# aarchiiive/diff-unet-amos

Measured on NVIDIA B200. Metric: 96^3 patches/s (DDIM-10), higher is better.
Workload: dtype fp16 (fp32 accumulate; encoder in split-bf16)

## Files before the change

### diff-unet-amos_b200/csrc/conv3d_ref.cuh

```cuda
#pragma once
#include <cuda_bf16.h>
#include <cuda_runtime.h>

#include "elementwise.cuh"

namespace dunet {

template <bool HF>
__global__ void __launch_bounds__(128) conv3d_ref_kernel(const __nv_bfloat16* __restrict__ src0, int c0, int chunks0,
                                                         const __nv_bfloat16* __restrict__ src1, int c1, int chunks1,
                                                         const float* __restrict__ w ,
                                                         __nv_bfloat16* __restrict__ out, int cout, int out_chunks,
                                                         int D, int H, int W, int batch, int rot) {
  const long long vox = (long long)D * H * W;
  const int och = (cout + 7) / 8;
  const int cin = c0 + c1;
  const long long total = (long long)batch * och * vox;
  for (long long i = blockIdx.x * (long long)blockDim.x + threadIdx.x; i < total;
       i += (long long)gridDim.x * blockDim.x) {
    const long long v = i % vox;
    const int oc = (int)((i / vox) % och);
    const int n = (int)(i / (vox * och));
    const int x = (int)(v % W), y = (int)((v / W) % H), z = (int)(v / ((long long)W * H));
    float acc[8];
#pragma unroll
    for (int j = 0; j < 8; ++j) acc[j] = 0.f;
    for (int tz = 0; tz < 3; ++tz) {
      const int zz = z + tz - 1;
      if (zz < 0 || zz >= D) continue;
      for (int ty = 0; ty < 3; ++ty) {
        const int yy = y + ty - 1;
        if (yy < 0 || yy >= H) continue;
        for (int tx = 0; tx < 3; ++tx) {
          const int xx = x + tx - 1;
          if (xx < 0 || xx >= W) continue;
          const int tap = (tz * 3 + ty) * 3 + tx;
          const long long sv = ((long long)zz * H + yy) * W + xx;
          for (int ci = 0; ci < cin; ci += 8) {
            const bool second = ci >= c0;
            const BF8* sp = second ? reinterpret_cast<const BF8*>(src1) + ((long long)n * chunks1 + (ci - c0) / 8) * vox
                                   : reinterpret_cast<const BF8*>(src0) + ((long long)n * chunks0 + ci / 8) * vox;
            float xi[8];
            bf8_to_float<HF>(sp[sv], xi);
#pragma unroll
            for (int k = 0; k < 8; ++k) {
              if (ci + k < cin) {
#pragma unroll
                for (int j = 0; j < 8; ++j) {
                  if (oc * 8 + j >= cout) continue;
                  const float wv =
                      round_16<HF>(w[((long long)(oc * 8 + j) * cin + (rot ? (ci + k + 1) % c0 : ci + k)) * 27 + tap]);
                  acc[j] = fmaf(xi[k], wv, acc[j]);
                }
              }
            }
          }
        }
      }
    }
    reinterpret_cast<BF8*>(out)[((long long)n * out_chunks + oc) * vox + v] = float_to_bf8<HF>(acc);
  }
}

}
```

### diff-unet-amos_b200/csrc/conv3d_tc64.cuh

```cuda
#pragma once
#include <cuda.h>
#include <cuda_bf16.h>
#include <cuda_runtime.h>

#include <type_traits>

#include "conv3d_tc.cuh"

namespace dunet {

template <int CB_CH, int ZT>
struct ConvTc64 {
  static constexpr int HX = CONV_TX + 2, HY = CONV_TY + 2;
  static constexpr int KCH = CB_CH / 8;
  static constexpr int KC = CB_CH / 16;
  static constexpr int PLANE_BYTES = KCH * HY * HX * 16;
  static constexpr int A_LBO = HY * HX * 16, A_SBO = HX * 16;
  static constexpr int NROWS = 192;
  static constexpr int W_UNIT_BYTES = KCH * NROWS * 16;
  static constexpr int B_LBO = NROWS * 16, B_SBO = 128;
  static constexpr int PLANES = ZT + 2;
  static constexpr int A_SLOTS = CB_CH == 32 ? 2 * PLANES + 1 : PLANES + 1;
  static constexpr int W_SLOTS = CB_CH == 32 ? 4 : 2;
  static constexpr int ACC_COLS = ZT * 64;
  static constexpr int TMEM_COLS = 512;
  static constexpr int RED_BYTES = 4 * 128 * 4;
  static constexpr int SMEM_BYTES = A_SLOTS * PLANE_BYTES + W_SLOTS * W_UNIT_BYTES + RED_BYTES + 1024 + 512;
  static constexpr int XFORM_WARPS = 8;
  static constexpr int THREADS_FUSED = CONV_THREADS + XFORM_WARPS * 32;
  static_assert(2 * ACC_COLS <= 512, "double-buffered accumulators exceed TMEM");
  static_assert(SMEM_BYTES <= 232448, "shared memory budget");
};

struct ConvTc64Args {
  const __nv_bfloat16* w;
  __nv_bfloat16* out;
  __nv_bfloat16* out_lo;
  float* stats;
  ConvSegs segs;
  int D, H, W;
  int tiles_x, tiles_y, tiles_z, batch;
  const float* in_affine;
  const float* in_bias;
  int in_bias_n_stride;
  float slope;
};

template <class F>
__device__ __forceinline__ void for_each_tile(int tiles_per_n, int batch, F&& f) {
  const int G = gridDim.x, shift = tiles_per_n % G;
  for (int n = 0; n < batch; ++n) {
    const int r = (int)((blockIdx.x + (long long)G * batch - (long long)n * shift) % G);
    for (int lin = r; lin < tiles_per_n; lin += G) f(n, lin);
  }
}

template <int CB_CH, int ZT, bool FUSE, bool H>
__global__ void __launch_bounds__(FUSE ? ConvTc64<CB_CH, ZT>::THREADS_FUSED : CONV_THREADS, 1)
conv3d_tc64_kernel(const __grid_constant__ CUtensorMap tmap0, const __grid_constant__ CUtensorMap tmap1,
                   const __grid_constant__ CUtensorMap tmap2, const __grid_constant__ CUtensorMap tmap3, ConvTc64Args a) {
  using Cfg = ConvTc64<CB_CH, ZT>;
  extern __shared__ uint8_t smem_raw[];
  const uint32_t smem_base = (smem_u32(smem_raw) + 1023u) & ~1023u;
  const uint32_t a_smem = smem_base;
  const uint32_t w_smem = a_smem + Cfg::A_SLOTS * Cfg::PLANE_BYTES;
  const uint32_t red_smem = w_smem + Cfg::W_SLOTS * Cfg::W_UNIT_BYTES;
  const uint32_t bars = red_smem + Cfg::RED_BYTES;
  const uint32_t a_full = bars, a_empty = bars + 8 * Cfg::A_SLOTS;
  const uint32_t w_full = bars + 16 * Cfg::A_SLOTS, w_empty = w_full + 8 * Cfg::W_SLOTS;
  const uint32_t acc_full = w_empty + 8 * Cfg::W_SLOTS;
  const uint32_t acc_empty = acc_full + 16;
  const uint32_t tmem_slot = acc_empty + 16;
  const uint32_t a_ready = tmem_slot + 8;
  static_assert(16 * Cfg::A_SLOTS + 16 * Cfg::W_SLOTS + 32 + 8 + 8 * Cfg::A_SLOTS <= 512, "barrier block");
  float* red = reinterpret_cast<float*>(smem_raw + (red_smem - smem_u32(smem_raw)));

  const int warp = threadIdx.x >> 5, lane = threadIdx.x & 31;
  const int ncb = a.segs.ncb;
  const int tiles_per_n = a.tiles_x * a.tiles_y * a.tiles_z;

  if (threadIdx.x == 0) {
    for (int i = 0; i < Cfg::A_SLOTS; ++i) { mbar_init(a_full + 8 * i, 1); mbar_init(a_empty + 8 * i, 1); mbar_init(a_ready + 8 * i, Cfg::XFORM_WARPS); }
    for (int i = 0; i < Cfg::W_SLOTS; ++i) { mbar_init(w_full + 8 * i, 1); mbar_init(w_empty + 8 * i, 1); }
    for (int i = 0; i < 2; ++i) { mbar_init(acc_full + 8 * i, 1); mbar_init(acc_empty + 8 * i, 4); }
    fence_mbar_init();
  }
  if (warp == 2) {
    tmem_alloc(tmem_slot, Cfg::TMEM_COLS);
    tmem_relinquish();
  }
  if (warp == 0 && lane == 0) {
    tma_prefetch_desc(&tmap0);
    if (a.segs.n > 1) tma_prefetch_desc(&tmap1);
    if (a.segs.n > 2) { tma_prefetch_desc(&tmap2); tma_prefetch_desc(&tmap3); }
  }
  tc_fence_before();
  __syncthreads();
  tc_fence_after();
  pdl_wait();
  uint32_t tmem_base;
  asm volatile("ld.shared.u32 %0, [%1];" : "=r"(tmem_base) : "r"(tmem_slot));

  if (warp == 0) {
    if (elect_one_sync()) {
      const CUtensorMap* const tms[4] = {&tmap0, &tmap1, &tmap2, &tmap3};
      int u = 0;
      for_each_tile(tiles_per_n, a.batch, [&](int n, int lin) {
        int t = lin;
        const int tix = t % a.tiles_x; t /= a.tiles_x;
        const int tiy = t % a.tiles_y; t /= a.tiles_y;
        const int tiz = t;
        const int x0 = tix * CONV_TX, y0 = tiy * CONV_TY, z0 = tiz * ZT;
        for (int cb = 0; cb < ncb; ++cb) {
          int ti, chunk0, chunks;
          conv_seg_lookup(a.segs, cb, Cfg::KCH, ti, chunk0, chunks);
          const CUtensorMap* tm = tms[ti];
          const int c3 = n * chunks + chunk0;
          for (int p = 0; p < Cfg::PLANES; ++p, ++u) {
            const int slot = u % Cfg::A_SLOTS, it = u / Cfg::A_SLOTS;
            if (it > 0) mbar_wait(a_empty + 8 * slot, (it - 1) & 1);
            mbar_arrive_expect_tx(a_full + 8 * slot, Cfg::PLANE_BYTES);
            tma_load_4d(a_smem + slot * Cfg::PLANE_BYTES, tm, a_full + 8 * slot, (x0 - 1) * 8, y0 - 1, z0 + p - 1, c3);
          }
        }
      });
    }
  } else if (warp == 1) {
    if (elect_one_sync()) {
      int w = 0;
      for_each_tile(tiles_per_n, a.batch, [&](int, int) {
        for (int i = 0; i < ncb * 9; ++i, ++w) {
          const int slot = w % Cfg::W_SLOTS, it = w / Cfg::W_SLOTS;
          if (it > 0) mbar_wait(w_empty + 8 * slot, (it - 1) & 1);
          mbar_arrive_expect_tx(w_full + 8 * slot, Cfg::W_UNIT_BYTES);
          bulk_load_1d(w_smem + slot * Cfg::W_UNIT_BYTES,
                       reinterpret_cast<const uint8_t*>(a.w) + (size_t)i * Cfg::W_UNIT_BYTES, Cfg::W_UNIT_BYTES,
                       w_full + 8 * slot);
        }
      });
    }
  } else if (warp == 2) {
    if (elect_one_sync()) {
      const uint64_t a_desc0 = make_smem_desc(a_smem, Cfg::A_LBO, Cfg::A_SBO);
      const uint64_t b_desc0 = make_smem_desc(w_smem, Cfg::B_LBO, Cfg::B_SBO);
      const uint32_t a_lo0 = (uint32_t)a_desc0, a_hi = (uint32_t)(a_desc0 >> 32);
      const uint32_t b_lo0 = (uint32_t)b_desc0, b_hi = (uint32_t)(b_desc0 >> 32);
      static_assert((Cfg::W_SLOTS & (Cfg::W_SLOTS - 1)) == 0, "W_SLOTS must be a power of two");
      int u0 = 0, w = 0, li = 0;
      for_each_tile(tiles_per_n, a.batch, [&](int, int) {
        const int buf = li & 1, use = li >> 1;
        if (use > 0) { mbar_wait(acc_empty + 8 * buf, (use - 1) & 1); tc_fence_after(); }
        const uint32_t acc = tmem_base + buf * Cfg::ACC_COLS;
        for (int cb = 0; cb < ncb; ++cb, u0 += Cfg::PLANES) {
          uint32_t pl_lo[Cfg::PLANES], pl_bar[Cfg::PLANES];
          uint32_t par[Cfg::PLANES];
#pragma unroll
          for (int p = 0; p < Cfg::PLANES; ++p) {
            const int u = u0 + p, slot = u % Cfg::A_SLOTS;
            pl_lo[p] = a_lo0 + slot * (Cfg::PLANE_BYTES >> 4);
            pl_bar[p] = 8 * slot;
            par[p] = (u / Cfg::A_SLOTS) & 1;
          }
          auto tap = [&](auto kind, int tyx, bool first_cb) {
            constexpr int KIND = decltype(kind)::value;
            const int ws = w & (Cfg::W_SLOTS - 1);
            mbar_wait(w_full + 8 * ws, (w / Cfg::W_SLOTS) & 1);
            tc_fence_after();
            const uint32_t tap16 = (tyx / 3) * Cfg::HX + (tyx % 3);
            const uint32_t bl_u = b_lo0 + ws * (Cfg::W_UNIT_BYTES >> 4);
#pragma unroll
            for (int p = 0; p < Cfg::PLANES; ++p) {
              if constexpr (KIND == 0) {
                mbar_wait((FUSE ? a_ready : a_full) + pl_bar[p], par[p]);
                tc_fence_after();
              }
              constexpr int dummy = 0; (void)dummy;
              const int slab_lo = p >= 2 ? p - 2 : 0, slab_hi = p < ZT ? p : ZT - 1;
              const int nblk = slab_hi - slab_lo + 1;
              const int row0 = (2 - (p - slab_lo)) * 64;
              const uint32_t al_p = pl_lo[p] + tap16, bl_p = bl_u + row0;
#pragma unroll
              for (int k = 0; k < Cfg::KC; ++k) {
                const uint32_t al = al_p + k * 2 * (Cfg::A_LBO >> 4), bl = bl_p + k * 2 * (Cfg::B_LBO >> 4);
                if (KIND == 0 && k == 0 && first_cb) {
#pragma unroll
                  for (int i = 0; i < nblk; ++i) {
                    const int sl = slab_lo + i, tz = p - sl;
                    umma_bf16_lh(acc + sl * 64, al, a_hi, bl + i * 64, b_hi, make_idesc_16(128, 64, H), tz != 0 ? 1u : 0u);
                  }
                } else {
                  umma_bf16_lh(acc + slab_lo * 64, al, a_hi, bl, b_hi, make_idesc_16(128, 64 * nblk, H), 1u);
                }
              }
              if constexpr (KIND == 2) umma_commit(a_empty + pl_bar[p]);
            }
            umma_commit(w_empty + 8 * ws);
            ++w;
          };
          tap(std::integral_constant<int, 0>{}, 0, cb == 0);
#pragma unroll 1
          for (int tyx = 1; tyx < 8; ++tyx) tap(std::integral_constant<int, 1>{}, tyx, false);
          tap(std::integral_constant<int, 2>{}, 8, false);
        }
        umma_commit(acc_full + 8 * buf);
        ++li;
      });
    }
    __syncwarp();
    pdl_trigger();
  } else if (FUSE && warp >= 7) {
    constexpr int LPC = Cfg::XFORM_WARPS * 32 / Cfg::KCH;
    constexpr int NPOS = Cfg::HY * Cfg::HX;
    constexpr int NV = (NPOS + LPC - 1) / LPC;
    const int tt = threadIdx.x - 7 * 32, chunk = tt / LPC, l0 = tt % LPC;
    uint8_t* const a_gen = smem_raw + (a_smem - smem_u32(smem_raw)) + chunk * (NPOS * 16) + l0 * 16;
    int pos_y[NV], pos_x[NV];
#pragma unroll
    for (int j = 0; j < NV; ++j) {
      const int i = l0 + j * LPC;
      pos_y[j] = i < NPOS ? i / Cfg::HX : 1 << 20;
      pos_x[j] = i % Cfg::HX;
    }
    float sc[8], sh[8], bi[8];
    int u = 0;
    for_each_tile(tiles_per_n, a.batch, [&](int n, int lin) {
      int t = lin;
      const int tix = t % a.tiles_x; t /= a.tiles_x;
      const int tiy = t % a.tiles_y; t /= a.tiles_y;
      const int tiz = t;
      const int x0 = tix * CONV_TX - 1, y0 = tiy * CONV_TY - 1, z0 = tiz * ZT - 1;
      uint32_t mask = 0;
#pragma unroll
      for (int j = 0; j < NV; ++j) {
        const int gy = y0 + pos_y[j], gx = x0 + pos_x[j];
        if (gy >= 0 && gy < a.H && gx >= 0 && gx < a.W) mask |= 1u << j;
      }
      for (int cb = 0; cb < ncb; ++cb) {
        {
          const int gch = cb * Cfg::KCH + chunk;
          const float4* src = reinterpret_cast<const float4*>(a.in_affine + ((long long)n * (ncb * Cfg::KCH) + gch) * 16);
#ifdef DUNET_AFFINE_LDG
          const float4 s0 = __ldg(src), s1 = __ldg(src + 1), h0 = __ldg(src + 2), h1 = __ldg(src + 3);
#else
          const float4 s0 = __ldcg(src), s1 = __ldcg(src + 1), h0 = __ldcg(src + 2), h1 = __ldcg(src + 3);
#endif
          sc[0] = s0.x; sc[1] = s0.y; sc[2] = s0.z; sc[3] = s0.w; sc[4] = s1.x; sc[5] = s1.y; sc[6] = s1.z; sc[7] = s1.w;
          sh[0] = h0.x; sh[1] = h0.y; sh[2] = h0.z; sh[3] = h0.w; sh[4] = h1.x; sh[5] = h1.y; sh[6] = h1.z; sh[7] = h1.w;
#pragma unroll
          for (int j = 0; j < 8; ++j) bi[j] = a.in_bias ? __ldg(a.in_bias + (long long)n * a.in_bias_n_stride + gch * 8 + j) : 0.f;
        }
        for (int p = 0; p < Cfg::PLANES; ++p, ++u) {
          const int slot = u % Cfg::A_SLOTS;
          mbar_wait(a_full + 8 * slot, (u / Cfg::A_SLOTS) & 1);
          const int gz = z0 + p;
          if (gz >= 0 && gz < a.D) {
            uint8_t* const pl = a_gen + slot * Cfg::PLANE_BYTES;
            constexpr int G = 6;
#pragma unroll
            for (int j0 = 0; j0 < NV; j0 += G) {
              BF8 v[G];
#pragma unroll
              for (int j = 0; j < G; ++j)
                if (j0 + j < NV && (mask >> (j0 + j) & 1u)) v[j] = *reinterpret_cast<const BF8*>(pl + (j0 + j) * (LPC * 16));
#pragma unroll
              for (int j = 0; j < G; ++j)
                if (j0 + j < NV && (mask >> (j0 + j) & 1u)) {
                  float f[8];
                  bf8_to_float<H>(v[j], f);
                  norm_apply(f, sc, sh, bi, a.slope);
                  *reinterpret_cast<BF8*>(pl + (j0 + j) * (LPC * 16)) = float_to_bf8<H>(f);
                }
            }
          }
          fence_proxy_async_smem();
          __syncwarp();
          if (lane == 0) mbar_arrive(a_ready + 8 * slot);
        }
      }
    });
  } else {
    const int q = warp & 3;
    const int r = q * 32 + lane;
    const long long vox = (long long)a.D * a.H * a.W;
    float run[4] = {0.f, 0.f, 0.f, 0.f};
    int cur_n = 0;
// ... 76 lines not shown
```

### diff-unet-amos_b200/csrc/dunet.cu

```cuda
#include <algorithm>
#include <atomic>
#include <cmath>
#include <cstdarg>
#include <cstdio>
#include <cstdlib>
#include <cstring>
#include <mutex>
#include <set>
#include <string>
#include <unordered_map>
#include <vector>

#include <cuda.h>
#include <cuda_bf16.h>
#include <cuda_runtime.h>

#include "../../include/dunet.h"
#include "conv3d_ref.cuh"
#include "conv3d_tc.cuh"
#include "conv3d_tc64.cuh"
#include "conv3d_flat.cuh"
#include "deconv2_tc.cuh"
#include "elementwise.cuh"
#include "surface.cuh"
// ... 58 lines not shown
}
static int prof_end_(Prof* pr, cudaStream_t st) {
  if (!pr || !pr->on) return 0;
  CUDA_TRY(cudaEventRecord(pr->recs[pr->used].b, st));
  ++pr->used;
  return 0;
}
#define prof_begin(tag, st) prof_begin_(prof_of(p), tag, st)
#define prof_end(st) prof_end_(prof_of(p), st)
#define PROF_ON (prof_of(p)->on)

template <typename... KArgs, typename... Args>
static void launch_k(void (*kern)(KArgs...), dim3 grid, dim3 block, size_t smem, cudaStream_t st, Args&&... args) {
  cudaLaunchConfig_t cfg;
  memset(&cfg, 0, sizeof cfg);
  cfg.gridDim = grid; cfg.blockDim = block; cfg.dynamicSmemBytes = smem; cfg.stream = st;
  cudaLaunchAttribute at[1];
  at[0].id = cudaLaunchAttributeProgrammaticStreamSerialization;
  at[0].val.programmaticStreamSerializationAllowed = 1;
  cfg.attrs = at; cfg.numAttrs = 1;
  (void)cudaLaunchKernelEx(&cfg, kern, std::forward<Args>(args)...);
}

static inline int pad_to(int v, int m) { return (v + m - 1) / m * m; }
static inline int grid_for(long long total, int threads, int cap = 148 * 16) {
  long long b = (total + threads - 1) / threads;
  if (b > cap) b = cap;
  if (b < 1) b = 1;
  return (int)b;
}
static bool aligned16(const void* p) { return (reinterpret_cast<uintptr_t>(p) & 15u) == 0; }

typedef CUresult (*EncodeTiledFn)(CUtensorMap*, CUtensorMapDataType, cuuint32_t, void*, const cuuint64_t*,
                                  const cuuint64_t*, const cuuint32_t*, const cuuint32_t*, CUtensorMapInterleave,
                                  CUtensorMapSwizzle, CUtensorMapL2promotion, CUtensorMapFloatOOBfill);
static EncodeTiledFn g_encode = nullptr;

static int load_driver_entry() {
  if (g_encode) return 0;
  void* fn = nullptr;
  cudaDriverEntryPointQueryResult q;
  CUDA_TRY(cudaGetDriverEntryPoint("cuTensorMapEncodeTiled", &fn, cudaEnableDefault, &q));
  if (!fn || q != cudaDriverEntryPointSuccess) return fail(DUNET_E_CUDA, "cuTensorMapEncodeTiled not available");
  g_encode = reinterpret_cast<EncodeTiledFn>(fn);
  return 0;
}

static int make_act_tmap(CUtensorMap* m, const bf16* base, int planes, int D, int H, int W, int kch, int halo) {
  TRY(load_driver_entry());
  cuuint64_t dims[4] = {(cuuint64_t)W * 8, (cuuint64_t)H, (cuuint64_t)D, (cuuint64_t)planes};
  cuuint64_t strides[3] = {(cuuint64_t)W * 16, (cuuint64_t)H * W * 16, (cuuint64_t)D * H * W * 16};
  cuuint32_t box[4] = {(cuuint32_t)(CONV_TX + 2 * halo) * 8, (cuuint32_t)(CONV_TY + 2 * halo), 1, (cuuint32_t)kch};
  cuuint32_t estr[4] = {1, 1, 1, 1};
  CUresult r = g_encode(m, CU_TENSOR_MAP_DATA_TYPE_BFLOAT16, 4, const_cast<bf16*>(base), dims, strides, box, estr,
                        CU_TENSOR_MAP_INTERLEAVE_NONE, CU_TENSOR_MAP_SWIZZLE_NONE, CU_TENSOR_MAP_L2_PROMOTION_L2_256B,
                        CU_TENSOR_MAP_FLOAT_OOB_FILL_NONE);
  if (r != CUDA_SUCCESS) return fail(DUNET_E_CUDA, "cuTensorMapEncodeTiled failed with CUresult %d (W=%d H=%d D=%d planes=%d)",
                                     (int)r, W, H, D, planes);
  return 0;
}

static int make_flat_tmap(CUtensorMap* m, const bf16* base, int planes, int D, int H, int W, int hx, int ty, int halo = 1) {
  TRY(load_driver_entry());
  cuuint64_t dims[4] = {(cuuint64_t)W * 8, (cuuint64_t)H, (cuuint64_t)D, (cuuint64_t)planes};
  cuuint64_t strides[3] = {(cuuint64_t)W * 16, (cuuint64_t)H * W * 16, (cuuint64_t)D * H * W * 16};
  cuuint32_t box[4] = {(cuuint32_t)hx * 8, (cuuint32_t)(ty + 2 * halo), 1, 8};
  cuuint32_t estr[4] = {1, 1, 1, 1};
  CUresult r = g_encode(m, CU_TENSOR_MAP_DATA_TYPE_BFLOAT16, 4, const_cast<bf16*>(base), dims, strides, box, estr,
                        CU_TENSOR_MAP_INTERLEAVE_NONE, CU_TENSOR_MAP_SWIZZLE_NONE, CU_TENSOR_MAP_L2_PROMOTION_L2_256B,
                        CU_TENSOR_MAP_FLOAT_OOB_FILL_NONE);
  if (r != CUDA_SUCCESS) return fail(DUNET_E_CUDA, "cuTensorMapEncodeTiled (flat) failed with CUresult %d (W=%d H=%d D=%d planes=%d hx=%d ty=%d)",
                                     (int)r, W, H, D, planes, hx, ty);
  return 0;
}

__device__ __forceinline__ bf16 weight_part(float v, int part, int fp16) {
  if (fp16) {
    const __half h = __float2half_rn(v);
    return *reinterpret_cast<const bf16*>(&h);
  }
  const bf16 hi = __float2bfloat16_rn(v);
  return part < 2 ? hi : __float2bfloat16_rn(v - __bfloat162float(hi));
}
__global__ void pack_conv_w_kernel(const float* __restrict__ w, bf16* __restrict__ out, int coutr, int cinr, int c0r,
                                   int c0p, int c1r, int cb_ch, int n_tile, int ncb, int n_tiles, int rot, int parts, int fp16, int triple) {
  const int kch = cb_ch / 8;
  const int ncb1 = ncb / parts;
  const long long total = (long long)n_tiles * ncb * 27 * kch * n_tile * 8;
  for (long long i = blockIdx.x * (long long)blockDim.x + threadIdx.x; i < total;
       i += (long long)gridDim.x * blockDim.x) {
    long long t = i;
    const int j = (int)(t % 8); t /= 8;
    const int col = (int)(t % n_tile); t /= n_tile;
    const int k = (int)(t % kch); t /= kch;
    const int tap = (int)(t % 27); t /= 27;
    const int cbg = (int)(t % ncb); t /= ncb;
    const int nt = (int)t;
    const int co = nt * n_tile + col;
    const int cb = cbg % ncb1, part = parts == 1 ? 0 : cbg / ncb1;
    const int lc = cb * cb_ch + k * 8 + j;
    int ci = -1, wpart = part;
    if (triple) {
      if (lc < 3 * c0r) { ci = lc % c0r; wpart = lc / c0r == 2 ? 2 : 0; }
    } else if (lc < c0p) { if (lc < c0r) ci = rot ? (lc + 1) % c0r : lc; }
    else { const int l1 = lc - c0p; if (l1 < c1r) ci = c0r + l1; }
    float v = 0.f;
    if (co < coutr && ci >= 0) v = w[((long long)co * cinr + ci) * 27 + tap];
    out[i] = weight_part(v, wpart, fp16);
  }
}
__global__ void pack_conv_w64_kernel(const float* __restrict__ w, bf16* __restrict__ out, int coutr, int cinr, int c0r,
                                     int c0p, int c1r, int cb_ch, int ncb, int rot, int parts, int fp16, int triple) {
  const int kch = cb_ch / 8;
  const int ncb1 = ncb / parts;
  const long long total = (long long)ncb * 9 * kch * 192 * 8;
  for (long long i = blockIdx.x * (long long)blockDim.x + threadIdx.x; i < total;
       i += (long long)gridDim.x * blockDim.x) {
    long long t = i;
    const int j = (int)(t % 8); t /= 8;
    const int row = (int)(t % 192); t /= 192;
    const int k = (int)(t % kch); t /= kch;
    const int tyx = (int)(t % 9); t /= 9;
    const int cbg = (int)t;
    const int cb = cbg % ncb1, part = parts == 1 ? 0 : cbg / ncb1;
    const int tz = 2 - row / 64, co = row % 64;
    const int tap = tz * 9 + tyx;
    const int lc = cb * cb_ch + k * 8 + j;
    int ci = -1, wpart = part;
    if (triple) {
      if (lc < 3 * c0r) { ci = lc % c0r; wpart = lc / c0r == 2 ? 2 : 0; }
    } else if (lc < c0p) { if (lc < c0r) ci = rot ? (lc + 1) % c0r : lc; }
    else { const int l1 = lc - c0p; if (l1 < c1r) ci = c0r + l1; }
    float v = 0.f;
    if (co < coutr && ci >= 0) v = w[((long long)co * cinr + ci) * 27 + tap];
    out[i] = weight_part(v, wpart, fp16);
  }
}
__global__ void pack_deconv_w_kernel(const float* __restrict__ w, bf16* __restrict__ out, int cinr, int coutr, int cinp,
                                     int coutp, int fp16) {
  const long long total = 8LL * cinp * coutp;
  for (long long i = blockIdx.x * (long long)blockDim.x + threadIdx.x; i < total;
       i += (long long)gridDim.x * blockDim.x) {
    const int co = (int)(i % coutp);
    const int ci = (int)((i / coutp) % cinp);
    const int tap = (int)(i / ((long long)coutp * cinp));
    float v = 0.f;
    if (ci < cinr && co < coutr) v = w[((long long)ci * coutr + co) * 8 + tap];
    out[i] = weight_part(v, 0, fp16);
  }
}
__global__ void pack_deconv_tc_w_kernel(const float* __restrict__ w, bf16* __restrict__ out, int cinr, int coutr, int cinp,
                                        int coutp, int parts, int fp16) {
  const int n_tile = 128, kch = 8, ncb1 = cinp / 64, ncb = ncb1 * parts, n_tiles = 8 * coutp / n_tile;
  const long long total = (long long)n_tiles * ncb * kch * n_tile * 8;
  for (long long i = blockIdx.x * (long long)blockDim.x + threadIdx.x; i < total;
       i += (long long)gridDim.x * blockDim.x) {
    long long t = i;
    const int j = (int)(t % 8); t /= 8;
    const int col = (int)(t % n_tile); t /= n_tile;
    const int k = (int)(t % kch); t /= kch;
    const int cbg = (int)(t % ncb); t /= ncb;
    const int nt = (int)t;
    const int cb = cbg % ncb1, part = parts == 1 ? 0 : cbg / ncb1;
    const int nblk = coutp / 64, dzdy = nt / nblk;
    const int tap = dzdy * 2 + col / 64, co = (nt - dzdy * nblk) * 64 + col % 64;
    const int ci = cb * 64 + k * 8 + j;
    float v = 0.f;
    if (ci < cinr && co < coutr) v = w[((long long)ci * coutr + co) * 8 + tap];
    out[i] = weight_part(v, part, fp16);
  }
}
__global__ void copy_pad_rows_kernel(const float* __restrict__ src, float* __restrict__ dst, int rows, int cols,
                                     int rows_pad, int cols_pad) {
  const long long total = (long long)rows_pad * cols_pad;
  for (long long i = blockIdx.x * (long long)blockDim.x + threadIdx.x; i < total;
       i += (long long)gridDim.x * blockDim.x) {
    const int c = (int)(i % cols_pad), r = (int)(i / cols_pad);
    dst[i] = (r < rows && c < cols) ? src[(long long)r * cols + c] : 0.f;
  }
}

struct ConvW {
  int c0r = 0, c1r = 0, c0p = 0, c1p = 0, coutr = 0, coutp = 0;
  int cb_ch = 64, n_tile = 64, nb0 = 0, nb1 = 0, n_tiles = 1;
  int parts = 1;
  bool split = false;
  bool triple = false;
  bf16* packed = nullptr;
  bf16* packed64 = nullptr;
  float* w32 = nullptr;
  float *gamma = nullptr, *beta = nullptr;
  int rot = 0;
  bool have_w = false, have_cb = false, have_g = false, have_b = false;
  void shape(int c0r_, int c0p_, int c1r_, int c1p_, int coutr_, int parts_ = 1, int cb64_ = 32) {
    c0r = c0r_; c0p = c0p_; c1r = c1r_; c1p = c1p_; coutr = coutr_; parts = parts_;
    split = parts_ == 3;
    triple = false;
    cb64 = (c1p == 0 && c0p == 32) ? 32 : cb64_;
    coutp = pad_to(coutr, 64);
    cb_ch = (c1p == 0 && c0p == 32) ? 32 : 64;
    n_tile = (coutp % 128 == 0) ? 128 : 64;
    n_tiles = coutp / n_tile;
    nb0 = c0p / cb_ch; nb1 = c1p / cb_ch;
  }
  int ncb() const { return (nb0 + nb1) * parts; }
  size_t packed_elems() const { return (size_t)n_tiles * ncb() * 27 * cb_ch * n_tile; }
  int cb64 = 32;
  int ncb64() const { return (c0p + c1p) / cb64 * parts; }
  size_t packed64_elems() const { return (size_t)ncb64() * 9 * cb64 * 192; }
};
struct Act {
  bf16* hi = nullptr;
  bf16* lo = nullptr;
};
struct TwoConvW {
  ConvW a, b;
  float *tp_w = nullptr, *tp_b = nullptr;
  bool has_temb = false, have_tpw = false, have_tpb = false;
};
struct DeconvW {
  int cinr = 0, cinp = 0, coutr = 0, coutp = 0, parts = 1;
  bf16* packed = nullptr;
  bf16* packed_tc = nullptr;
  float* bias = nullptr;
  bool have_w = false, have_b = false;
};

enum SlotKind { K_CONV_W, K_CONV_B, K_IN_G, K_IN_B, K_TP_W, K_TP_B, K_DENSE, K_DECONV_W, K_DECONV_B, K_FINAL_W, K_FINAL_B };
struct Slot {
  SlotKind kind;
  void* obj;
  int idx;
  std::vector<int64_t> shape;
  bool seen = false;
};

struct WsLayout {
  size_t in_pack, raw, mid, partial, ss, splitk, affine, x_t, acc, image, total;
  size_t emb[5], epool[5], x[5], dpool[5], up[5], u[5];
};

struct dunet_plan {
  dunet_cfg cfg;
  int C, D[5], H[5], W[5];
  long long V[5];
  int fr[6], fp[6];
  int upr[5], upp[5];
  int uoutr[5], uoutp[5];
  int in_pad = 32;
  TwoConvW enc[5], den[5], upc[5];
  DeconvW dec[5];
  float* dense[4] = {nullptr, nullptr, nullptr, nullptr};
  float *final_w = nullptr, *final_b = nullptr;
  std::unordered_map<std::string, Slot> slots;
  int n_steps = 0;
  std::vector<int> tmap;
  std::vector<float> sr, srm1, acp;
  int* d_tmap = nullptr;
  float* temb_table = nullptr;
  int temb_row = 0, temb_off[9];
  bool committed = false;
  int emb_B = 0;
  bool emb_dual = false;
  std::vector<void*> owned;
  cudaStream_t half_stream[2] = {nullptr, nullptr};
  cudaEvent_t ev_fork = nullptr, ev_join[2] = {nullptr, nullptr};
  int num_sms = 0;
  mutable Prof prof;
  static constexpr int T_RING = 8;
  int* h_t = nullptr;
  int* d_t = nullptr;
  float* temb_scratch = nullptr;
  cudaEvent_t t_ev[T_RING] = {};
  int t_slot = 0;
};
static Prof* prof_of(const dunet_plan* p) { return &p->prof; }

static int dev_alloc(dunet_plan* p, void** out, size_t bytes) {
  CUDA_TRY(cudaMalloc(out, bytes ? bytes : 16));
  p->owned.push_back(*out);
  return 0;
}

static void add_slot(dunet_plan* p, const std::string& key, SlotKind kind, void* obj, std::vector<int64_t> shape, int idx = 0) {
  Slot s; s.kind = kind; s.obj = obj; s.idx = idx; s.shape = std::move(shape);
  p->slots[key] = s;
}
static void add_convblock_slots(dunet_plan* p, const std::string& pre, ConvW* c) {
  add_slot(p, pre + ".conv.weight", K_CONV_W, c, {c->coutr, c->c0r + c->c1r, 3, 3, 3});
  add_slot(p, pre + ".conv.bias", K_CONV_B, c, {c->coutr});
  add_slot(p, pre + ".adn.N.weight", K_IN_G, c, {c->coutr});
  add_slot(p, pre + ".adn.N.bias", K_IN_B, c, {c->coutr});
}
// ... 116 lines not shown

static inline bool is_prec(const dunet_plan* p) { return (p->cfg.flags & DUNET_FLAG_FP32X3) != 0; }
static inline bool is_fp16(const dunet_plan* p) { return (p->cfg.flags & DUNET_FLAG_FP16) != 0; }
#define DUNET_FMT(cond, ...)                               \
  do {                                                     \
    if (cond) { constexpr bool HF = true; __VA_ARGS__; }   \
    else { constexpr bool HF = false; __VA_ARGS__; }       \
  } while (0)
struct BiasRef {
  const float* p = nullptr;
  int n_stride = 0;
  BiasRef at(int off) const { BiasRef r; r.p = p ? p + off : nullptr; r.n_stride = n_stride; return r; }
};
static inline Act ws_act_x(const dunet_plan* p, uint8_t* ws, size_t off, int ch, int lvl, int B, bool prec) {
  Act a;
  a.hi = reinterpret_cast<bf16*>(ws + off);
  a.lo = prec ? a.hi + (size_t)B * ch * (size_t)p->V[lvl] : nullptr;
  return a;
}
static inline Act ws_act(const dunet_plan* p, uint8_t* ws, size_t off, int ch, int lvl, int B) {
  return ws_act_x(p, ws, off, ch, lvl, B, is_prec(p));
}
static inline bool enc_prec(const dunet_plan* p) {
  return is_prec(p) || (is_fp16(p) && !(p->cfg.flags & (DUNET_FLAG_PLAIN_ENCODER | DUNET_FLAG_REF_CONV)));
}
static inline bool fmt_h(const dunet_plan* p, bool prec) { return is_fp16(p) && !prec; }

static WsLayout ws_layout(const dunet_plan* p, int B) {
  WsLayout L;
  size_t off = 0;
  const size_t pm = is_prec(p) ? 2 : 1, pme = enc_prec(p) ? 2 : 1;
  auto take = [&](size_t bytes) { size_t o = off; off += (bytes + 255) / 256 * 256; return o; };
  auto act_m = [&](int ch, int lvl, size_t m) -> size_t { return (size_t)(m * (size_t)B * ch * (size_t)p->V[lvl] * sizeof(bf16)); };
  auto act = [&](int ch, int lvl) -> size_t { return act_m(ch, lvl, pm); };
  L.in_pack = take(act_m(p->in_pad, 0, std::max(pm, pme)));
  size_t raw_max = 0, part_max = 0, ss_max = 0, split_max = 0;
  auto upd = [&](const ConvW& c, int lvl) {
    raw_max = std::max(raw_max, act_m(c.coutp, lvl, c.split ? 2 : 1));
    const ConvPlan g = conv_plan(p, c, lvl, true);
    const size_t planes = (size_t)B * (c.coutp / 8);
    part_max = std::max(part_max, planes * std::max(g.tiles, 160) * 16 * sizeof(float));
    ss_max = std::max(ss_max, planes * 16 * sizeof(float));
    if (g.ksplit > 1) split_max = std::max(split_max, (size_t)g.ksplit * B * c.coutp * (size_t)p->V[lvl] * sizeof(float));
  };
  for (int l = 0; l < 5; ++l) { upd(p->enc[l].a, l); upd(p->enc[l].b, l); upd(p->den[l].a, l); upd(p->den[l].b, l); }
  for (int l = 4; l >= 1; --l) { upd(p->upc[l].a, l - 1); upd(p->upc[l].b, l - 1); }
  L.raw = take(raw_max);
  L.mid = take(raw_max);
  L.partial = take(part_max);
  L.ss = take(ss_max);
  L.splitk = take(split_max);
  L.affine = take(ss_max);
  const int CP = p->C <= 8 ? 8 : (p->C <= 16 ? 16 : 32);
  L.x_t = take((size_t)B * CP * p->V[0] * sizeof(float));
  L.acc = take((size_t)B * CP * p->V[0] * sizeof(float));
  L.image = take((size_t)B * p->cfg.in_channels * p->V[0] * sizeof(float));
  for (int l = 0; l < 5; ++l) {
    L.emb[l] = take(act(p->fp[l], l));
    L.x[l] = take(act(p->fp[l], l));
    L.epool[l] = l ? take(act_m(p->fp[l - 1], l, pme)) : 0;
    L.dpool[l] = l ? take(act(p->fp[l - 1], l)) : 0;
    L.up[l] = l ? take(act(p->upp[l], l - 1)) : 0;
    L.u[l] = l ? take(act(p->uoutp[l], l - 1)) : 0;
  }
  L.total = off;
  return L;
}

static long long* g_conv_dbg = nullptr;
static int g_conv_dbg_count = 0;

#define DUNET_TC_KERNELS_H(X, H)                                                                  \
  X((conv3d_tc_kernel<32, 64, CONV_ZT, MODE_CONV3, H>), (ConvTc<32, 64, CONV_ZT, MODE_CONV3>::SMEM_BYTES))     \
  X((conv3d_tc_kernel<32, 128, CONV_ZT, MODE_CONV3, H>), (ConvTc<32, 128, CONV_ZT, MODE_CONV3>::SMEM_BYTES))   \
  X((conv3d_tc_kernel<64, 64, 2, MODE_CONV3, H>), (ConvTc<64, 64, 2, MODE_CONV3>::SMEM_BYTES))                 \
  X((conv3d_tc_kernel<64, 128, 2, MODE_CONV3, H>), (ConvTc<64, 128, 2, MODE_CONV3>::SMEM_BYTES))               \
  X((conv3d_tc_kernel<64, 64, CONV_ZT, MODE_CONV3, H>), (ConvTc<64, 64, CONV_ZT, MODE_CONV3>::SMEM_BYTES))     \
  X((conv3d_tc_kernel<64, 128, CONV_ZT, MODE_CONV3, H>), (ConvTc<64, 128, CONV_ZT, MODE_CONV3>::SMEM_BYTES))   \
  X((conv3d_tc_kernel<64, 128, 2, MODE_DECONV2, H>), (ConvTc<64, 128, 2, MODE_DECONV2>::SMEM_BYTES))           \
  X((conv3d_tc64_kernel<32, CONV_ZT, false, H>), (ConvTc64<32, CONV_ZT>::SMEM_BYTES))                          \
  X((conv3d_tc64_kernel<32, CONV_ZT, true, H>), (ConvTc64<32, CONV_ZT>::SMEM_BYTES))                           \
  X((conv3d_tc64_kernel<64, CONV_ZT, false, H>), (ConvTc64<64, CONV_ZT>::SMEM_BYTES))                          \
  X((conv3d_tc64_kernel<64, CONV_ZT, true, H>), (ConvTc64<64, CONV_ZT>::SMEM_BYTES))                           \
  X((deconv2_tc_kernel<1, 2, H>), (DeconvTc<1, 2>::SMEM_BYTES))                                                \
  X((deconv2_tc_kernel<2, 2, H>), (DeconvTc<2, 2>::SMEM_BYTES))                                                \
  X((conv3d_flat_kernel<1, H>), FLAT_SMEM_MAX)                                                                 \
  X((conv3d_flat_kernel<2, H>), FLAT_SMEM_MAX)                                                                 \
  X((conv3d_flat_kernel<3, H>), FLAT_SMEM_MAX)                                                                 \
  X((conv3d_flat_kernel<4, H>), FLAT_SMEM_MAX)                                                                 \
  X((conv3d_flat_kernel<6, H>), FLAT_SMEM_MAX)

static std::mutex g_dev_mu;
static std::unordered_map<int, int> g_dev_sms;
static int dev_prepare(int* sms_out) {
  int dev = 0;
  CUDA_TRY(cudaGetDevice(&dev));
  std::lock_guard<std::mutex> lock(g_dev_mu);
  auto it = g_dev_sms.find(dev);
  if (it == g_dev_sms.end()) {
    int sms = 0;
    CUDA_TRY(cudaDeviceGetAttribute(&sms, cudaDevAttrMultiProcessorCount, dev));
#define DUNET_SET_SMEM(K, BYTES) CUDA_TRY(cudaFuncSetAttribute(K, cudaFuncAttributeMaxDynamicSharedMemorySize, BYTES));
    DUNET_TC_KERNELS_H(DUNET_SET_SMEM, false)
    DUNET_TC_KERNELS_H(DUNET_SET_SMEM, true)
#undef DUNET_SET_SMEM
    it = g_dev_sms.emplace(dev, sms).first;
  }
  if (sms_out) *sms_out = it->second;
  return 0;
}

template <int CB_CH, int N_TILE, int ZT, int MODE, bool H>
static int launch_conv_tc(const dunet_plan* p, const CUtensorMap (&t)[4], const ConvTcArgs& a, cudaStream_t st, int conv_tag = PROF_CONV) {
  using Cfg = ConvTc<CB_CH, N_TILE, ZT, MODE>;
  auto kern = conv3d_tc_kernel<CB_CH, N_TILE, ZT, MODE, H>;
  const long long items = (long long)a.tiles_x * a.tiles_y * a.tiles_z * a.n_tiles * a.ksplit * a.batch;
  const long long grid = std::min<long long>(items, (long long)p->num_sms);
  TRY(prof_begin(conv_tag, st));
  launch_k(kern, dim3((unsigned)grid), dim3(CONV_TC_THREADS), Cfg::SMEM_BYTES, st, t[0], t[1], t[2], t[3], a);
  LAUNCH_CHECK();
  TRY(prof_end(st));
  return 0;
}

template <int CB_CH, bool FUSE, bool H>
static int launch_conv_tc64(const dunet_plan* p, const CUtensorMap (&t)[4], const ConvTc64Args& a, unsigned* grid_out, cudaStream_t st,
                            int conv_tag = PROF_CONV) {
  using Cfg = ConvTc64<CB_CH, CONV_ZT>;
  auto kern = conv3d_tc64_kernel<CB_CH, CONV_ZT, FUSE, H>;
  const long long tiles = (long long)a.tiles_x * a.tiles_y * a.tiles_z * a.batch;
  const unsigned grid = (unsigned)std::min<long long>(tiles, p->num_sms);
  *grid_out = grid;
  TRY(prof_begin(conv_tag, st));
  launch_k(kern, dim3(grid), dim3(FUSE ? Cfg::THREADS_FUSED : CONV_THREADS), Cfg::SMEM_BYTES, st, t[0], t[1], t[2], t[3], a);
  LAUNCH_CHECK();
  TRY(prof_end(st));
  return 0;
}

static int launch_flat(const dunet_plan* p, const CUtensorMap (&t)[4], ConvFlatArgs f, const FlatGeom& g, bool h, int tag, cudaStream_t st) {
  f.hx = g.hx; f.ty = g.ty; f.tiles_y = g.tiles_y; f.tiles_z = g.tiles_z;
  f.npos = g.npos; f.lbo = g.lbo; f.a_slots = g.a_slots; f.w_slots = g.w_slots;
  const long long items = (long long)f.tiles_y * f.tiles_z * f.n_tiles * f.ksplit * f.batch;
  const unsigned grid = (unsigned)std::min<long long>(items, p->num_sms);
  TRY(prof_begin(tag, st));
  DUNET_FMT(h, {
    switch (g.zt) {
      case 1: launch_k(conv3d_flat_kernel<1, HF>, dim3(grid), dim3(FLAT_THREADS), (size_t)g.smem, st, t[0], t[1], t[2], t[3], f); break;
      case 2: launch_k(conv3d_flat_kernel<2, HF>, dim3(grid), dim3(FLAT_THREADS), (size_t)g.smem, st, t[0], t[1], t[2], t[3], f); break;
      case 3: launch_k(conv3d_flat_kernel<3, HF>, dim3(grid), dim3(FLAT_THREADS), (size_t)g.smem, st, t[0], t[1], t[2], t[3], f); break;
      case 4: launch_k(conv3d_flat_kernel<4, HF>, dim3(grid), dim3(FLAT_THREADS), (size_t)g.smem, st, t[0], t[1], t[2], t[3], f); break;
      default: launch_k(conv3d_flat_kernel<6, HF>, dim3(grid), dim3(FLAT_THREADS), (size_t)g.smem, st, t[0], t[1], t[2], t[3], f); break;
    }
  });
  LAUNCH_CHECK();
  TRY(prof_end(st));
  return 0;
}

static long long* conv_dbg_stamp() {
  static const int target = [] { const char* e = getenv("DUNET_DBG_LAUNCH"); return e ? atoi(e) : -1; }();
  long long* dbg = (g_conv_dbg && (target < 0 || g_conv_dbg_count == target)) ? g_conv_dbg : nullptr;
  if (g_conv_dbg) ++g_conv_dbg_count;
  return dbg;
}

static ConvSegs make_segs(int nb0, int chunks0, int nb1, int chunks1, bool prec) {
  ConvSegs sg;
  memset(&sg, 0, sizeof sg);
  auto add = [&](int tm, int nb, int chunks) {
    if (nb > 0) { sg.s[sg.n].tmap = tm; sg.s[sg.n].nblocks = nb; sg.s[sg.n].chunks = chunks; ++sg.n; sg.ncb += nb; }
  };
  add(0, nb0, chunks0); add(1, nb1, chunks1);
  if (prec) { add(2, nb0, chunks0); add(3, nb1, chunks1); add(0, nb0, chunks0); add(1, nb1, chunks1); }
  return sg;
}

struct FuseIn {
  const float* affine = nullptr;
  BiasRef bias;
};

static bool splitk_norm_ok(const dunet_plan* p, bool prec, int lvl) {
  return !prec && p->V[lvl] <= SKN_MAX_VOX && p->D[lvl] % 2 == 0 && p->H[lvl] % 2 == 0 && p->W[lvl] % 2 == 0;
}
static int run_conv(const dunet_plan* p, const ConvW& c, const ConvPlan& cp, Act src0, Act src1, Act out, float* partial,
                    float* splitk, int* nseg_out, int lvl, int B, cudaStream_t st, const FuseIn* fuse = nullptr,
                    int* pending_split = nullptr) {
  if (pending_split) *pending_split = 0;
  const int D = p->D[lvl], H = p->H[lvl], W = p->W[lvl];
  const int planes = B * (c.coutp / 8);
  const bool prec = c.split, pairs_in = prec && !c.triple;
  if (prec && (!out.lo || (pairs_in && (!src0.lo || (c.nb1 > 0 && !src1.lo))))) return fail(DUNET_E_STATE, "split-precision conv needs hi + lo tensors");
  if (fuse && !cp.fuse_input) return fail(DUNET_E_STATE, "normalise-on-load requested for a conv that cannot take it");
  if (cp.ksplit > 1 && (!partial || !splitk)) return fail(DUNET_E_STATE, "K-split conv without partial-tile buffers");
  if (cp.kernel == CONV_REF) {
    if (prec) return fail(DUNET_E_UNSUPPORTED, "DUNET_FLAG_REF_CONV and DUNET_FLAG_FP32X3 are mutually exclusive");
    if (!c.w32) return fail(DUNET_E_STATE, "DUNET_FLAG_REF_CONV needs DUNET_FLAG_KEEP_FP32_WEIGHTS");
    CUDA_TRY(cudaMemsetAsync(out.hi, 0, (size_t)B * c.coutp * p->V[lvl] * sizeof(bf16), st));
    DUNET_FMT(fmt_h(p, prec), conv3d_ref_kernel<HF><<<grid_for((long long)B * ((c.coutr + 7) / 8) * p->V[lvl], 128, 148 * 64), 128, 0, st>>>(
        src0.hi, c.c0r, c.c0p / 8, src1.hi, c.c1r, c.c1p / 8, c.w32, out.hi, c.coutr, c.coutp / 8, D, H, W, B, c.rot));
    LAUNCH_CHECK();
    if (partial) {
      const int nseg = stats_nseg(p->V[lvl]);
      DUNET_FMT(fmt_h(p, prec), in_stats_kernel<HF><<<dim3(nseg, planes), STATS_THREADS, 0, st>>>(out.hi, partial, p->V[lvl], nseg));
      LAUNCH_CHECK();
      *nseg_out = nseg;
    }
    return 0;
  }
  const int conv_tag = (prec && !is_prec(p)) ? PROF_CONV_SPLIT : PROF_CONV;
  if (PROF_ON) {
    const double fl = 2.0 * B * (double)p->V[lvl] * c.coutr * 27.0 * (c.c0r + c.c1r);
    prof_of(p)->bytes[conv_tag] += fl;
    if (conv_tag == PROF_CONV) prof_of(p)->flops += fl;
  }
  const ConvSegs segs = make_segs(c.c0p / cp.cb, c.c0p / 8, c.c1p / cp.cb, c.c1p / 8, pairs_in);
  auto tmap = [&](CUtensorMap* m, const bf16* base, int ch) {
    return cp.kernel == CONV_FLAT ? make_flat_tmap(m, base, B * (ch / 8), D, H, W, cp.flat.hx, cp.flat.ty)
                                  : make_act_tmap(m, base, B * (ch / 8), D, H, W, cp.cb / 8, 1);
  };
  CUtensorMap t[4];
  TRY(tmap(&t[0], src0.hi, c.c0p));
  t[1] = t[2] = t[3] = t[0];
  if (c.nb1 > 0) TRY(tmap(&t[1], src1.hi, c.c1p));
  if (pairs_in) {
    TRY(tmap(&t[2], src0.lo, c.c0p));
    if (c.nb1 > 0) TRY(tmap(&t[3], src1.lo, c.c1p));
  }
  switch (cp.kernel) {
    case CONV_TC64: {
      if (!c.packed64) return fail(DUNET_E_STATE, "conv weights not packed for the Cout = 64 kernel");
      ConvTc64Args b;
      memset(&b, 0, sizeof b);
      b.w = c.packed64; b.out = out.hi; b.out_lo = out.lo; b.stats = partial; b.segs = segs;
      b.D = D; b.H = H; b.W = W; b.tiles_x = cp.tiles_x; b.tiles_y = cp.tiles_y; b.tiles_z = cp.tiles_z; b.batch = B;
      unsigned grid = 0;
      if (fuse) {
        b.in_affine = fuse->affine; b.in_bias = fuse->bias.p; b.in_bias_n_stride = fuse->bias.n_stride; b.slope = 0.1f;
        DUNET_FMT(fmt_h(p, prec), TRY(cp.cb == 32 ? (launch_conv_tc64<32, true, HF>(p, t, b, &grid, st, conv_tag)) : (launch_conv_tc64<64, true, HF>(p, t, b, &grid, st, conv_tag))));
      } else {
        DUNET_FMT(fmt_h(p, prec), TRY(cp.cb == 32 ? (launch_conv_tc64<32, false, HF>(p, t, b, &grid, st, conv_tag)) : (launch_conv_tc64<64, false, HF>(p, t, b, &grid, st, conv_tag))));
      }
      if (partial) *nseg_out = (int)grid;
      return 0;
    }
    case CONV_FLAT: {
      ConvFlatArgs f;
      memset(&f, 0, sizeof f);
      f.w = c.packed; f.out = out.hi; f.out_lo = out.lo; f.segs = segs;
      f.cout = c.coutp; f.D = D; f.H = H; f.W = W; f.n_tiles = c.n_tiles; f.batch = B;
      f.ksplit = cp.ksplit; f.ksub = cp.ksub;
      f.dbg = conv_dbg_stamp();
      if (cp.ksplit > 1) f.out_partial = splitk;
      else f.stats = partial;
      TRY(launch_flat(p, t, f, cp.flat, fmt_h(p, prec), conv_tag, st));
      break;
    }
    default: {
      ConvTcArgs a;
      memset(&a, 0, sizeof a);
      a.w = c.packed; a.out = out.hi; a.out_lo = out.lo; a.segs = segs;
      a.cout = c.coutp; a.D = D; a.H = H; a.W = W;
      a.tiles_x = cp.tiles_x; a.tiles_y = cp.tiles_y; a.tiles_z = cp.tiles_z; a.n_tiles = c.n_tiles; a.batch = B;
      a.ksplit = cp.ksplit;
      a.dbg = conv_dbg_stamp();
      if (cp.ksplit > 1) a.out_partial = splitk;
      else a.stats = partial;
      int rc = 0;
      DUNET_FMT(fmt_h(p, prec), {
        if (c.cb_ch == 32 && c.n_tile == 64) rc = launch_conv_tc<32, 64, CONV_ZT, MODE_CONV3, HF>(p, t, a, st, conv_tag);
        else if (c.cb_ch == 32 && c.n_tile == 128) rc = launch_conv_tc<32, 128, CONV_ZT, MODE_CONV3, HF>(p, t, a, st, conv_tag);
        else if (c.cb_ch == 64 && c.n_tile == 64 && cp.zt == 2) rc = launch_conv_tc<64, 64, 2, MODE_CONV3, HF>(p, t, a, st, conv_tag);
        else if (c.cb_ch == 64 && c.n_tile == 128 && cp.zt == 2) rc = launch_conv_tc<64, 128, 2, MODE_CONV3, HF>(p, t, a, st, conv_tag);
        else if (c.cb_ch == 64 && c.n_tile == 64) rc = launch_conv_tc<64, 64, CONV_ZT, MODE_CONV3, HF>(p, t, a, st, conv_tag);
        else if (c.cb_ch == 64 && c.n_tile == 128) rc = launch_conv_tc<64, 128, CONV_ZT, MODE_CONV3, HF>(p, t, a, st, conv_tag);
        else rc = fail(DUNET_E_UNSUPPORTED, "no conv instantiation for cb_ch=%d n_tile=%d", c.cb_ch, c.n_tile);
      });
      TRY(rc);
      break;
    }
  }
  if (cp.ksplit == 1) {
    if (partial) *nseg_out = cp.tiles;
    return 0;
  }
  if (pending_split && splitk_norm_ok(p, prec, lvl)) {
    *pending_split = cp.ksplit;
    *nseg_out = 0;
    return 0;
  }
  const int nseg = (int)std::min<long long>(std::max<long long>((p->V[lvl] + 255) / 256, 1), 128);
  if (PROF_ON) prof_of(p)->bytes[PROF_SPLITK] += (double)B * c.coutp * (double)p->V[lvl] * (4.0 * cp.ksplit + (prec ? 4.0 : 2.0));
  TRY(prof_begin(PROF_SPLITK, st));
  DUNET_FMT(fmt_h(p, prec), launch_k(splitk_reduce_stats_kernel<HF>, dim3(nseg, planes), dim3(STATS_THREADS), 0, st, (const float*)splitk, cp.ksplit,
           (long long)B * c.coutp * p->V[lvl], out.hi, out.lo, partial, (long long)p->V[lvl], nseg));
  LAUNCH_CHECK();
  TRY(prof_end(st));
  *nseg_out = nseg;
  return 0;
}

static int run_norm(const dunet_plan* p, const ConvW& c, Act raw, const float* partial, int nseg, BiasRef bias, Act add,
                    Act out, Act pooled, int lvl, int B, cudaStream_t st, int pending_split = 0, const float* splitk = nullptr) {
  const int planes = B * (c.coutp / 8);
  const bool prec = raw.lo != nullptr;
  NormActArgs a;
  memset(&a, 0, sizeof a);
  a.raw = raw.hi; a.partial = partial; a.nseg = nseg; a.gamma = c.gamma; a.beta = c.beta; a.bias = bias.p; a.bias_n_stride = bias.n_stride; a.add = add.hi;
  a.out = out.hi; a.pooled = pooled.hi; a.raw_lo = raw.lo; a.add_lo = add.lo; a.out_lo = out.lo; a.pooled_lo = pooled.lo;
  a.chunks = c.coutp / 8; a.D = p->D[lvl]; a.H = p->H[lvl]; a.W = p->W[lvl];
  a.eps = 1e-5f; a.slope = 0.1f;
  if (pending_split > 1) {
    if (prec || !splitk || add.lo || p->V[lvl] > SKN_MAX_VOX) return fail(DUNET_E_STATE, "fused split-K normalise: unsupported configuration");
    SplitkNormArgs k;
    k.part = splitk; k.ksplit = pending_split; k.split_stride = (long long)B * c.coutp * p->V[lvl]; k.n = a;
    if (PROF_ON) prof_of(p)->bytes[PROF_NORM_SMALL] += (double)B * c.coutp * (double)p->V[lvl] * (4.0 * pending_split + 2.0 + (add.hi ? 2.0 : 0.0) + (pooled.hi ? 0.25 : 0.0));
    TRY(prof_begin(PROF_NORM_SMALL, st));
#define DUNET_SKN(ADDF, POOLF) DUNET_FMT(is_fp16(p), launch_k(splitk_norm_kernel<ADDF, POOLF, HF>, dim3(planes), dim3(256), 0, st, k))
    if (add.hi && pooled.hi) DUNET_SKN(true, true);
    else if (add.hi) DUNET_SKN(true, false);
// ... 109 lines not shown
      b.tiles_x = (W + CONV_TX - 1) / CONV_TX; b.tiles_y = (H + CONV_TY - 1) / CONV_TY; b.tiles_z = (D + 1) / 2;
      b.n_tiles = 8 * d.coutp / 128; b.batch = B; b.dbg = getenv("DUNET_DBG_DECONV") ? g_conv_dbg : nullptr;
      const long long tiles = (long long)b.tiles_x * b.tiles_y * b.tiles_z * B;
      const unsigned grid = (unsigned)std::min<long long>(tiles, p->num_sms);
      TRY(prof_begin(dtag, st));
      if (d.cinp == 64) DUNET_FMT(is_fp16(p), launch_k(deconv2_tc_kernel<1, 2, HF>, dim3(grid), dim3(DeconvTc<1, 2>::THREADS), DeconvTc<1, 2>::SMEM_BYTES, st, t[0], b));
      else DUNET_FMT(is_fp16(p), launch_k(deconv2_tc_kernel<2, 2, HF>, dim3(grid), dim3(DeconvTc<2, 2>::THREADS), DeconvTc<2, 2>::SMEM_BYTES, st, t[0], b));
      LAUNCH_CHECK();
      TRY(prof_end(st));
      return 0;
    }
    case DECONV_FLAT: {
      TRY(make_flat_tmap(&t[0], in.hi, B * (d.cinp / 8), D, H, W, dp.flat.hx, dp.flat.ty, 0));
      t[1] = t[2] = t[3] = t[0];
      ConvFlatArgs f;
      memset(&f, 0, sizeof f);
      f.w = d.packed_tc; f.out = out.hi; f.bias = d.bias; f.deconv = 1;
      f.segs = make_segs(d.cinp / 64, d.cinp / 8, 0, 0, false);
      f.cout = d.coutp; f.D = D; f.H = H; f.W = W; f.n_tiles = 8 * d.coutp / 128; f.batch = B; f.ksplit = 1; f.ksub = 1;
      return launch_flat(p, t, f, dp.flat, is_fp16(p), dtag, st);
    }
    default: {
      TRY(make_act_tmap(&t[0], in.hi, B * (d.cinp / 8), D, H, W, 8, 0));
      t[1] = t[2] = t[3] = t[0];
      if (prec) TRY(make_act_tmap(&t[1], in.lo, B * (d.cinp / 8), D, H, W, 8, 0));
      ConvTcArgs a;
      memset(&a, 0, sizeof a);
      a.w = d.packed_tc; a.out = out.hi; a.out_lo = out.lo; a.bias = d.bias;
      a.segs = make_segs(d.cinp / 64, d.cinp / 8, 0, 0, false);
      if (prec) {
        a.segs.n = 3; a.segs.ncb = 3 * (d.cinp / 64);
        a.segs.s[1] = a.segs.s[0]; a.segs.s[1].tmap = 1;
        a.segs.s[2] = a.segs.s[0];
      }
      a.cout = d.coutp; a.D = D; a.H = H; a.W = W;
      a.tiles_x = (W + CONV_TX - 1) / CONV_TX; a.tiles_y = (H + CONV_TY - 1) / CONV_TY; a.tiles_z = (D + 1) / 2;
      a.n_tiles = 8 * d.coutp / 128; a.ksplit = 1; a.batch = B; a.dbg = nullptr;
      int rc = 0;
      DUNET_FMT(fmt_h(p, prec), rc = launch_conv_tc<64, 128, 2, MODE_DECONV2, HF>(p, t, a, st, dtag));
      return rc;
    }
  }
}

struct SubBatches {
  int n, B0;
  size_t ws_stride;
};
static SubBatches sub_batches(const dunet_plan* p, int B, bool dual) {
  SubBatches s;
  s.n = dual ? 2 : 1;
  s.B0 = (B + s.n - 1) / s.n;
  s.ws_stride = ws_layout(p, s.B0).total;
  return s;
}
static bool dual_batch(const dunet_plan* p, int B) { return B >= 4 && (p->cfg.flags & DUNET_FLAG_DUAL_STREAM); }
static bool use_dual(dunet_plan* p, int B, int run_encoder) {
  const bool dual = run_encoder ? (dual_batch(p, B) && !PROF_ON) : (p->emb_dual && p->emb_B == B);
  if (run_encoder) { p->emb_B = B; p->emb_dual = dual; }
  return dual;
}
template <typename Body>
static int run_sub_batches(dunet_plan* p, const SubBatches& s, int B, uint8_t* ws, cudaStream_t st, Body&& body) {
  if (s.n == 1) return body(0, B, ws, st);
  CUDA_TRY(cudaEventRecord(p->ev_fork, st));
  for (int h = 0; h < s.n; ++h) {
    CUDA_TRY(cudaStreamWaitEvent(p->half_stream[h], p->ev_fork, 0));
    TRY(body(h * s.B0, std::min(s.B0, B - h * s.B0), ws + h * s.ws_stride, p->half_stream[h]));
    CUDA_TRY(cudaEventRecord(p->ev_join[h], p->half_stream[h]));
  }
  for (int h = 0; h < s.n; ++h) CUDA_TRY(cudaStreamWaitEvent(st, p->ev_join[h], 0));
  return 0;
}

static int check_call(const dunet_plan* p, int B, const void* ws) {
  if (!p) return fail(DUNET_E_INVALID, "plan is NULL");
  if (!p->committed) return fail(DUNET_E_STATE, "plan not committed (dunet_plan_commit)");
  if (B < 1 || B > p->cfg.batch_max) return fail(DUNET_E_INVALID, "batch %d outside [1, %d]", B, p->cfg.batch_max);
  if (!ws || (reinterpret_cast<uintptr_t>(ws) & 255u)) return fail(DUNET_E_INVALID, "workspace must be non-NULL and 256-byte aligned");
  return 0;
}

static int launch_pack(const dunet_plan* p, const float* src0, int c0, const float* src1, int c1, Act dst, int c_pad,
                       long long vox, int B, cudaStream_t st, bool triple = false) {
  DUNET_FMT(fmt_h(p, dst.lo != nullptr || triple), launch_k(pack_c8_kernel<HF>, dim3(grid_for((long long)B * (c_pad / 8) * vox, 256)), dim3(256), 0, st,
                                 src0, c0, src1, c1, dst.hi, dst.lo, c_pad, vox, B, triple ? 1 : 0));
  LAUNCH_CHECK();
  return 0;
}

static int encode_impl(dunet_plan* p, const float* image, int B, uint8_t* ws, const WsLayout& L, cudaStream_t st) {
  const bool ep = enc_prec(p), triple = p->enc[0].a.triple;
  const Act in_pack = ws_act_x(p, ws, L.in_pack, p->in_pad, 0, B, ep && !triple);
  TRY(launch_pack(p, image, p->cfg.in_channels, nullptr, 0, in_pack, p->in_pad, p->V[0], B, st, triple));
  for (int l = 0; l < 5; ++l) {
    const Act src = l ? ws_act_x(p, ws, L.epool[l], p->fp[l - 1], l, B, ep) : in_pack;
    const Act pooled = l < 4 ? ws_act_x(p, ws, L.epool[l + 1], p->fp[l], l + 1, B, ep) : Act();
    TRY(run_twoconv(p, p->enc[l], src, Act(), BiasRef(), Act(), ws_act(p, ws, L.emb[l], p->fp[l], l, B), pooled, l, B, ws, L, st));
  }
  return 0;
}

static int unet_body(dunet_plan* p, BiasRef temb_row, int B, uint8_t* ws, const WsLayout& L, cudaStream_t st,
                     int* last_nseg, Act* last_raw) {
  const Act in_pack = ws_act(p, ws, L.in_pack, p->in_pad, 0, B);
  for (int l = 0; l < 5; ++l) {
    const Act src = l ? ws_act(p, ws, L.dpool[l], p->fp[l - 1], l, B) : in_pack;
    const Act pooled = l < 4 ? ws_act(p, ws, L.dpool[l + 1], p->fp[l], l + 1, B) : Act();
    TRY(run_twoconv(p, p->den[l], src, Act(), temb_row.at(p->temb_off[l]), ws_act(p, ws, L.emb[l], p->fp[l], l, B),
                    ws_act(p, ws, L.x[l], p->fp[l], l, B), pooled, l, B, ws, L, st));
  }
  Act prev = ws_act(p, ws, L.x[4], p->fp[4], 4, B);
  for (int l = 4; l >= 1; --l) {
    const Act up = ws_act(p, ws, L.up[l], p->upp[l], l - 1, B);
    TRY(run_deconv(p, p->dec[l], prev, up, l, B, st));
    const Act u = ws_act(p, ws, L.u[l], p->uoutp[l], l - 1, B);
    TRY(run_twoconv(p, p->upc[l], ws_act(p, ws, L.x[l - 1], p->fp[l - 1], l - 1, B), up, temb_row.at(p->temb_off[5 + (4 - l)]),
                    Act(), u, Act(), l - 1, B, ws, L, st, l == 1, last_nseg, l == 1 ? last_raw : nullptr));
    prev = u;
  }
  return 0;
}

static int launch_temb(dunet_plan* p, const int* d_t, int rows, float* table, cudaStream_t st) {
  TembArgs a;
  a.w0 = p->dense[0]; a.b0 = p->dense[1]; a.w1 = p->dense[2]; a.b1 = p->dense[3];
  const TwoConvW* blocks[9] = {&p->den[0], &p->den[1], &p->den[2], &p->den[3], &p->den[4],
                               &p->upc[4], &p->upc[3], &p->upc[2], &p->upc[1]};
  for (int i = 0; i < 9; ++i) {
    a.pw[i] = blocks[i]->tp_w; a.pb[i] = blocks[i]->tp_b; a.pc[i] = blocks[i]->a.coutr; a.poff[i] = p->temb_off[i];
  }
  a.row = p->temb_row; a.tmap = d_t; a.table = table;
  temb_table_kernel<<<rows, 512, 0, st>>>(a);
  LAUNCH_CHECK();
  return 0;
}

static void final_args_common(dunet_plan* p, FinalDdimArgs& a, uint8_t* ws, const WsLayout& L, int nseg, int B, Act feat) {
  (void)ws; (void)L;
  memset(&a, 0, sizeof a);
  a.feat = feat.hi; a.feat_lo = feat.lo; a.F = p->fp[5]; a.w = p->final_w; a.b = p->final_b; a.C = p->C;
  a.partial = reinterpret_cast<float*>(ws + L.partial); a.nseg = nseg; a.gamma = p->upc[1].b.gamma; a.beta = p->upc[1].b.beta;
  a.eps = 1e-5f; a.slope = 0.1f; a.in_pad = p->in_pad; a.vox = p->V[0]; a.batch = B;
}

static int launch_final(dunet_plan* p, const FinalDdimArgs& a, cudaStream_t st) {
  const dim3 grid(grid_for((a.vox + 15) / 16 * 32, FINAL_THREADS, std::max(1, 148 * 3 / a.batch)), a.batch);
  if (a.F != 64 && a.F != 128) return fail(DUNET_E_UNSUPPORTED, "final conv: padded features[5] must be 64 or 128");
  const bool prec = a.feat_lo != nullptr;
#define DUNET_FINAL(NT)                                                                            \
  do {                                                                                             \
    if (prec) {                                                                                    \
      if (a.F == 64) launch_k(final_ddim_kernel<NT, 4, MODE_FP32X3>, grid, dim3(FINAL_THREADS), 0, st, a);     \
      else launch_k(final_ddim_kernel<NT, 8, MODE_FP32X3>, grid, dim3(FINAL_THREADS), 0, st, a);               \
    } else if (is_fp16(p)) {                                                                       \
      if (a.F == 64) launch_k(final_ddim_kernel<NT, 4, MODE_FP16>, grid, dim3(FINAL_THREADS), 0, st, a);       \
      else launch_k(final_ddim_kernel<NT, 8, MODE_FP16>, grid, dim3(FINAL_THREADS), 0, st, a);                 \
    } else {                                                                                       \
      if (a.F == 64) launch_k(final_ddim_kernel<NT, 4, MODE_BF16>, grid, dim3(FINAL_THREADS), 0, st, a);       \
      else launch_k(final_ddim_kernel<NT, 8, MODE_BF16>, grid, dim3(FINAL_THREADS), 0, st, a);                 \
    }                                                                                              \
  } while (0)
  if (PROF_ON)
    prof_of(p)->bytes[PROF_FINAL] += (double)a.batch * (double)a.vox * ((prec ? 4.0 : 2.0) * a.F + (a.x_t ? 16.0 * a.C : 0.0) + (a.logits_out ? 4.0 * a.C : 0.0) + (a.next_in ? 2.0 * a.C : 0.0));
  TRY(prof_begin(PROF_FINAL, st));
  if (a.C <= 8) DUNET_FINAL(1);
  else if (a.C <= 16) DUNET_FINAL(2);
  else DUNET_FINAL(4);
#undef DUNET_FINAL
  LAUNCH_CHECK();
  TRY(prof_end(st));
  return 0;
}

struct Hd95Layout {
  size_t meta, off1, stack, off2, keys, total;
};
// ... 87 lines not shown
  *conv_ms = total; *conv_launches = n; *conv_flops = pr->flops;
  return 0;
}

int dunet_profile_read_all(dunet_plan* p, double* ms_by_tag, uint64_t* launches_by_tag, double* bytes_by_tag) {
  if (!p || !ms_by_tag || !launches_by_tag) return fail(DUNET_E_INVALID, "NULL argument");
  Prof* pr = prof_of(p);
  for (int i = 0; i < PROF_TAGS; ++i) { ms_by_tag[i] = 0.0; launches_by_tag[i] = 0; if (bytes_by_tag) bytes_by_tag[i] = pr->bytes[i]; }
  for (size_t i = 0; i < pr->used; ++i) {
    CUDA_TRY(cudaEventSynchronize(pr->recs[i].b));
    float ms = 0.f;
    CUDA_TRY(cudaEventElapsedTime(&ms, pr->recs[i].a, pr->recs[i].b));
    ms_by_tag[pr->recs[i].tag] += ms;
    launches_by_tag[pr->recs[i].tag] += 1;
  }
  return 0;
}

int dunet_profile_dump(dunet_plan* p, double* ms, int32_t* tags, int32_t capacity, int32_t* count) {
  if (!p || !ms || !tags || !count) return fail(DUNET_E_INVALID, "NULL argument");
  Prof* pr = prof_of(p);
  int n = 0;
  for (size_t i = 0; i < pr->used && n < capacity; ++i, ++n) {
    CUDA_TRY(cudaEventSynchronize(pr->recs[i].b));
    float t = 0.f;
    CUDA_TRY(cudaEventElapsedTime(&t, pr->recs[i].a, pr->recs[i].b));
    ms[n] = t; tags[n] = pr->recs[i].tag;
  }
  *count = n;
  return 0;
}

int dunet_debug_barrier_timeouts(uint32_t* out_flag) {
  if (!out_flag) return fail(DUNET_E_INVALID, "out_flag is NULL");
  CUDA_TRY(cudaMemcpyFromSymbol(out_flag, g_barrier_timeout_flag, sizeof(uint32_t)));
  return 0;
}

int dunet_plan_create(dunet_plan** out, const dunet_cfg* cfg) {
  if (!out || !cfg) return fail(DUNET_E_INVALID, "NULL argument");
  int ndev = 0;
  CUDA_TRY(cudaGetDeviceCount(&ndev));
  int dev = 0;
  CUDA_TRY(cudaGetDevice(&dev));
  cudaDeviceProp prop;
  CUDA_TRY(cudaGetDeviceProperties(&prop, dev));
  if (prop.major != 10) return fail(DUNET_E_UNSUPPORTED, "libdunet_b200 needs an sm_100a device (found sm_%d%d); there is no fallback path", prop.major, prop.minor);
  if (cfg->in_channels != 1) return fail(DUNET_E_UNSUPPORTED, "only in_channels == 1 is implemented");
  if (cfg->num_classes < 1 || cfg->num_classes + cfg->in_channels > 32 || cfg->num_classes > FINAL_MAX_C)
    return fail(DUNET_E_UNSUPPORTED, "num_classes must be in [1, 31]");
  for (int d = 0; d < 3; ++d)
    if (cfg->patch[d] < 32 || cfg->patch[d] % 16) return fail(DUNET_E_INVALID, "patch edge %d must be a multiple of 16 and >= 32", cfg->patch[d]);
  for (int i = 0; i < 6; ++i)
    if (cfg->features[i] < 1 || cfg->features[i] > 2048) return fail(DUNET_E_INVALID, "features[%d] = %d out of range", i, cfg->features[i]);
  if (cfg->features[4] % 2 || cfg->features[3] % 2 || cfg->features[2] % 2)
    return fail(DUNET_E_INVALID, "features[2..4] must be even (UpCat halves the channels)");
  if (cfg->batch_max < 1 || cfg->num_steps < 1 || cfg->num_steps > 1000) return fail(DUNET_E_INVALID, "bad batch_max / num_steps");
  if (pad_to(cfg->features[5], 64) > FINAL_MAX_F) return fail(DUNET_E_UNSUPPORTED, "features[5] > %d not implemented", FINAL_MAX_F);

  if ((cfg->flags & DUNET_FLAG_FP32X3) && (cfg->flags & DUNET_FLAG_REF_CONV))
    return fail(DUNET_E_UNSUPPORTED, "DUNET_FLAG_REF_CONV and DUNET_FLAG_FP32X3 are mutually exclusive");
  if ((cfg->flags & DUNET_FLAG_FP32X3) && (cfg->flags & DUNET_FLAG_FP16))
    return fail(DUNET_E_UNSUPPORTED, "DUNET_FLAG_FP16 and DUNET_FLAG_FP32X3 are mutually exclusive (the hi/lo split is bf16)");
  int sms = 0;
  TRY(dev_prepare(&sms));
  dunet_plan* p = new dunet_plan();
  p->cfg = *cfg;
  p->num_sms = sms;
  const int parts = (cfg->flags & DUNET_FLAG_FP32X3) ? 3 : 1;
  const int parts_enc = enc_prec(p) ? 3 : 1;
  const int cb64 = (cfg->flags & DUNET_FLAG_TC64_CB64) ? 64 : 32;
  p->C = cfg->num_classes;
  for (int l = 0; l < 5; ++l) {
    p->D[l] = cfg->patch[0] >> l; p->H[l] = cfg->patch[1] >> l; p->W[l] = cfg->patch[2] >> l;
    p->V[l] = (long long)p->D[l] * p->H[l] * p->W[l];
  }
  for (int i = 0; i < 6; ++i) { p->fr[i] = cfg->features[i]; p->fp[i] = pad_to(cfg->features[i], 64); }
  for (int l = 4; l >= 1; --l) {
    p->upr[l] = (l == 1) ? p->fr[1] : p->fr[l] / 2;
    p->upp[l] = pad_to(p->upr[l], 64);
    p->uoutr[l] = (l == 1) ? p->fr[5] : p->fr[l - 1];
    p->uoutp[l] = pad_to(p->uoutr[l], 64);
  }
  for (int l = 0; l < 5; ++l) {
    TwoConvW& e = p->enc[l];
    if (l == 0) {
      e.a.shape(cfg->in_channels, p->in_pad, 0, 0, p->fr[0], parts_enc, cb64);
      if (e.a.split && 3 * cfg->in_channels <= 32 && !(cfg->flags & DUNET_FLAG_REF_CONV)) {
        e.a.shape(cfg->in_channels, p->in_pad, 0, 0, p->fr[0], 1, cb64);
        e.a.split = true; e.a.triple = true;
      }
    } else e.a.shape(p->fr[l - 1], p->fp[l - 1], 0, 0, p->fr[l], parts_enc, cb64);
    e.b.shape(p->fr[l], p->fp[l], 0, 0, p->fr[l], parts_enc, cb64);
    TwoConvW& d = p->den[l];
    d.has_temb = true;
    if (l == 0) { d.a.shape(cfg->in_channels + p->C, p->in_pad, 0, 0, p->fr[0], parts, cb64); d.a.rot = 1; }
    else d.a.shape(p->fr[l - 1], p->fp[l - 1], 0, 0, p->fr[l], parts, cb64);
    d.b.shape(p->fr[l], p->fp[l], 0, 0, p->fr[l], parts, cb64);
  }
  for (int l = 4; l >= 1; --l) {
    TwoConvW& u = p->upc[l];
    u.has_temb = true;
    u.a.shape(p->fr[l - 1], p->fp[l - 1], p->upr[l], p->upp[l], p->uoutr[l], parts, cb64);
    u.b.shape(p->uoutr[l], p->uoutp[l], 0, 0, p->uoutr[l], parts, cb64);
    DeconvW& d = p->dec[l];
    d.cinr = p->fr[l]; d.cinp = p->fp[l]; d.coutr = p->upr[l]; d.coutp = p->upp[l]; d.parts = parts;
  }
  add_twoconv_slots(p, "embed_model.conv_0", &p->enc[0]);
  for (int l = 1; l < 5; ++l) add_twoconv_slots(p, "embed_model.down." + std::to_string(l - 1) + ".convs", &p->enc[l]);
  add_slot(p, "model.temb.dense.0.weight", K_DENSE, p, {512, 128}, 0);
  add_slot(p, "model.temb.dense.0.bias", K_DENSE, p, {512}, 1);
  add_slot(p, "model.temb.dense.1.weight", K_DENSE, p, {512, 512}, 2);
  add_slot(p, "model.temb.dense.1.bias", K_DENSE, p, {512}, 3);
  add_twoconv_slots(p, "model.conv_0", &p->den[0]);
  for (int l = 1; l < 5; ++l) add_twoconv_slots(p, "model.down_" + std::to_string(l) + ".convs", &p->den[l]);
  for (int l = 4; l >= 1; --l) {
    const std::string pre = "model.upcat_" + std::to_string(l);
    add_slot(p, pre + ".upsample.deconv.weight", K_DECONV_W, &p->dec[l], {p->dec[l].cinr, p->dec[l].coutr, 2, 2, 2});
    add_slot(p, pre + ".upsample.deconv.bias", K_DECONV_B, &p->dec[l], {p->dec[l].coutr});
    add_twoconv_slots(p, pre + ".convs", &p->upc[l]);
  }
  add_slot(p, "model.final_conv.weight", K_FINAL_W, p, {p->C, p->fr[5], 1, 1, 1});
  add_slot(p, "model.final_conv.bias", K_FINAL_B, p, {p->C});
  {
    const TwoConvW* blocks[9] = {&p->den[0], &p->den[1], &p->den[2], &p->den[3], &p->den[4],
                                 &p->upc[4], &p->upc[3], &p->upc[2], &p->upc[1]};
    int off = 0;
    for (int i = 0; i < 9; ++i) { p->temb_off[i] = off; off += blocks[i]->a.coutp; }
    p->temb_row = off;
  }
  *out = p;
  return 0;
}

void dunet_plan_destroy(dunet_plan* p) {
  if (!p) return;
  for (cudaStream_t s : p->half_stream)
    if (s) cudaStreamSynchronize(s);
  for (void* q : p->owned) cudaFree(q);
  if (p->h_t) cudaFreeHost(p->h_t);
  for (cudaEvent_t e : p->t_ev) if (e) cudaEventDestroy(e);
  for (ProfRec& r : p->prof.recs) { cudaEventDestroy(r.a); cudaEventDestroy(r.b); }
  for (int i = 0; i < 2; ++i) {
    if (p->half_stream[i]) cudaStreamDestroy(p->half_stream[i]);
    if (p->ev_join[i]) cudaEventDestroy(p->ev_join[i]);
  }
  if (p->ev_fork) cudaEventDestroy(p->ev_fork);
  delete p;
}

int dunet_plan_set_weight(dunet_plan* p, const char* key, const float* src, const int64_t* shape, int32_t ndim, void* stream) {
  if (!p || !key || !src || !shape) return fail(DUNET_E_INVALID, "NULL argument");
  cudaStream_t st = static_cast<cudaStream_t>(stream);
  auto it = p->slots.find(key);
  if (it == p->slots.end()) return fail(DUNET_E_INVALID, "unexpected checkpoint key '%s'", key);
  Slot& s = it->second;
  if ((int)s.shape.size() != ndim) return fail(DUNET_E_INVALID, "key '%s': expected %zu dims, got %d", key, s.shape.size(), ndim);
  for (int i = 0; i < ndim; ++i)
    if (s.shape[i] != shape[i]) return fail(DUNET_E_INVALID, "key '%s': dim %d is %lld, expected %lld", key, i, (long long)shape[i], (long long)s.shape[i]);
  if (!aligned16(src)) return fail(DUNET_E_INVALID, "key '%s': pointer not 16-byte aligned", key);
  p->committed = false;
  switch (s.kind) {
    case K_CONV_W: {
      ConvW* c = static_cast<ConvW*>(s.obj);
      if (!c->packed) TRY(dev_alloc(p, (void**)&c->packed, c->packed_elems() * sizeof(bf16)));
      const int cinr = c->c0r + c->c1r;
      pack_conv_w_kernel<<<grid_for((long long)c->packed_elems(), 256), 256, 0, st>>>(
          src, c->packed, c->coutr, cinr, c->c0r, c->c0p, c->c1r, c->cb_ch, c->n_tile, c->ncb(), c->n_tiles, c->rot, c->parts, fmt_h(p, c->split) ? 1 : 0, c->triple ? 1 : 0);
      LAUNCH_CHECK();
      if (c->coutp == 64) {
        const size_t n64 = c->packed64_elems();
        if (!c->packed64) TRY(dev_alloc(p, (void**)&c->packed64, n64 * sizeof(bf16)));
        pack_conv_w64_kernel<<<grid_for((long long)n64, 256), 256, 0, st>>>(src, c->packed64, c->coutr, cinr, c->c0r, c->c0p,
                                                                             c->c1r, c->cb64, c->ncb64(), c->rot, c->parts, fmt_h(p, c->split) ? 1 : 0, c->triple ? 1 : 0);
        LAUNCH_CHECK();
      }
      if (p->cfg.flags & DUNET_FLAG_KEEP_FP32_WEIGHTS) {
        const size_t bytes = (size_t)c->coutr * cinr * 27 * sizeof(float);
        if (!c->w32) TRY(dev_alloc(p, (void**)&c->w32, bytes));
        CUDA_TRY(cudaMemcpyAsync(c->w32, src, bytes, cudaMemcpyDeviceToDevice, st));
      }
      c->have_w = true;
      break;
    }
    case K_CONV_B:
      static_cast<ConvW*>(s.obj)->have_cb = true;
      break;
    case K_IN_G:
    case K_IN_B: {
      ConvW* c = static_cast<ConvW*>(s.obj);
      float** dst = s.kind == K_IN_G ? &c->gamma : &c->beta;
      if (!*dst) TRY(dev_alloc(p, (void**)dst, c->coutp * sizeof(float)));
      copy_pad_rows_kernel<<<1, 256, 0, st>>>(src, *dst, 1, c->coutr, 1, c->coutp);
      LAUNCH_CHECK();
      (s.kind == K_IN_G ? c->have_g : c->have_b) = true;
      break;
    }
    case K_TP_W:
    case K_TP_B: {
      TwoConvW* t = static_cast<TwoConvW*>(s.obj);
      const size_t n = s.kind == K_TP_W ? (size_t)t->a.coutr * 512 : (size_t)t->a.coutr;
      float** dst = s.kind == K_TP_W ? &t->tp_w : &t->tp_b;
      if (!*dst) TRY(dev_alloc(p, (void**)dst, n * sizeof(float)));
      CUDA_TRY(cudaMemcpyAsync(*dst, src, n * sizeof(float), cudaMemcpyDeviceToDevice, st));
      (s.kind == K_TP_W ? t->have_tpw : t->have_tpb) = true;
      break;
    }
    case K_DENSE: {
      size_t n = 1;
      for (auto d : s.shape) n *= (size_t)d;
      if (!p->dense[s.idx]) TRY(dev_alloc(p, (void**)&p->dense[s.idx], n * sizeof(float)));
      CUDA_TRY(cudaMemcpyAsync(p->dense[s.idx], src, n * sizeof(float), cudaMemcpyDeviceToDevice, st));
      break;
    }
    case K_DECONV_W: {
      DeconvW* d = static_cast<DeconvW*>(s.obj);
      const size_t n = 8ull * d->cinp * d->coutp;
      if (!d->packed) TRY(dev_alloc(p, (void**)&d->packed, n * sizeof(bf16)));
      pack_deconv_w_kernel<<<grid_for((long long)n, 256), 256, 0, st>>>(src, d->packed, d->cinr, d->coutr, d->cinp, d->coutp, is_fp16(p) ? 1 : 0);
      LAUNCH_CHECK();
      if (!d->packed_tc) TRY(dev_alloc(p, (void**)&d->packed_tc, n * d->parts * sizeof(bf16)));
      pack_deconv_tc_w_kernel<<<grid_for((long long)n * d->parts, 256), 256, 0, st>>>(src, d->packed_tc, d->cinr, d->coutr, d->cinp,
                                                                                      d->coutp, d->parts, is_fp16(p) ? 1 : 0);
      LAUNCH_CHECK();
      d->have_w = true;
      break;
    }
    case K_DECONV_B: {
      DeconvW* d = static_cast<DeconvW*>(s.obj);
      if (!d->bias) TRY(dev_alloc(p, (void**)&d->bias, d->coutp * sizeof(float)));
      copy_pad_rows_kernel<<<1, 256, 0, st>>>(src, d->bias, 1, d->coutr, 1, d->coutp);
      LAUNCH_CHECK();
      d->have_b = true;
      break;
    }
    case K_FINAL_W: {
      if (!p->final_w) TRY(dev_alloc(p, (void**)&p->final_w, (size_t)p->C * p->fp[5] * sizeof(float)));
      copy_pad_rows_kernel<<<grid_for((long long)p->C * p->fp[5], 256), 256, 0, st>>>(src, p->final_w, p->C, p->fr[5], p->C, p->fp[5]);
      LAUNCH_CHECK();
      break;
    }
    case K_FINAL_B: {
      if (!p->final_b) TRY(dev_alloc(p, (void**)&p->final_b, p->C * sizeof(float)));
      CUDA_TRY(cudaMemcpyAsync(p->final_b, src, p->C * sizeof(float), cudaMemcpyDeviceToDevice, st));
      break;
    }
  }
  s.seen = true;
  return 0;
}

int dunet_plan_set_schedule(dunet_plan* p, int32_t n, const int32_t* tmap, const float* sr, const float* srm1, const float* acp) {
  if (!p || !tmap || !sr || !srm1 || !acp) return fail(DUNET_E_INVALID, "NULL argument");
  if (n != p->cfg.num_steps) return fail(DUNET_E_INVALID, "schedule has %d steps, plan was created for %d", n, p->cfg.num_steps);
  p->n_steps = n;
  p->tmap.assign(tmap, tmap + n);
  p->sr.assign(sr, sr + n); p->srm1.assign(srm1, srm1 + n); p->acp.assign(acp, acp + n);
// ... 18 lines not shown
    TRY(dev_alloc(p, (void**)&p->d_t, (size_t)p->cfg.batch_max * sizeof(int)));
    TRY(dev_alloc(p, (void**)&p->temb_scratch, (size_t)p->cfg.batch_max * p->temb_row * sizeof(float)));
    CUDA_TRY(cudaMallocHost((void**)&p->h_t, (size_t)dunet_plan::T_RING * p->cfg.batch_max * sizeof(int)));
    for (int i = 0; i < dunet_plan::T_RING; ++i) CUDA_TRY(cudaEventCreateWithFlags(&p->t_ev[i], cudaEventDisableTiming));
  }
  if (!p->half_stream[0]) {
    for (int i = 0; i < 2; ++i) {
      CUDA_TRY(cudaStreamCreateWithFlags(&p->half_stream[i], cudaStreamNonBlocking));
      CUDA_TRY(cudaEventCreateWithFlags(&p->ev_join[i], cudaEventDisableTiming));
    }
    CUDA_TRY(cudaEventCreateWithFlags(&p->ev_fork, cudaEventDisableTiming));
  }
  CUDA_TRY(cudaStreamSynchronize(st));
  p->committed = true;
  return 0;
}

int dunet_workspace_bytes(const dunet_plan* p, int32_t batch, size_t* out) {
  if (!p || !out) return fail(DUNET_E_INVALID, "NULL argument");
  if (batch < 1 || batch > p->cfg.batch_max) return fail(DUNET_E_INVALID, "batch %d outside [1, %d]", batch, p->cfg.batch_max);
  const SubBatches s = sub_batches(p, batch, dual_batch(p, batch));
  *out = std::max(ws_layout(p, batch).total, s.n * s.ws_stride);
  return 0;
}

int dunet_encode(dunet_plan* p, const float* image, int32_t B, void* workspace, void* stream) {
  TRY(check_call(p, B, workspace));
  if (!image || !aligned16(image)) return fail(DUNET_E_INVALID, "image must be a 16-byte aligned device pointer");
  p->emb_B = B; p->emb_dual = false;
  return encode_impl(p, image, B, static_cast<uint8_t*>(workspace), ws_layout(p, B), static_cast<cudaStream_t>(stream));
}

int dunet_get_embedding(dunet_plan* p, int32_t level, float* out, int32_t B, void* workspace, void* stream) {
  TRY(check_call(p, B, workspace));
  if (level < 0 || level > 4 || !out) return fail(DUNET_E_INVALID, "bad level / NULL out");
  const WsLayout L = ws_layout(p, B);
  const Act e = ws_act(p, static_cast<uint8_t*>(workspace), L.emb[level], p->fp[level], level, B);
  DUNET_FMT(fmt_h(p, e.lo != nullptr), unpack_c8_kernel<HF><<<grid_for((long long)B * (p->fp[level] / 8) * p->V[level], 256), 256, 0, static_cast<cudaStream_t>(stream)>>>(
      e.hi, e.lo, p->fp[level], out, p->fr[level], p->V[level], B));
  LAUNCH_CHECK();
  return 0;
}

int dunet_set_embedding(dunet_plan* p, int32_t level, const float* in, int32_t B, void* workspace, void* stream) {
  TRY(check_call(p, B, workspace));
  if (level < 0 || level > 4 || !in) return fail(DUNET_E_INVALID, "bad level / NULL in");
  p->emb_B = B; p->emb_dual = false;
  const WsLayout L = ws_layout(p, B);
  return launch_pack(p, in, p->fr[level], nullptr, 0, ws_act(p, static_cast<uint8_t*>(workspace), L.emb[level], p->fp[level], level, B),
                     p->fp[level], p->V[level], B, static_cast<cudaStream_t>(stream));
}

int dunet_denoise_step(dunet_plan* p, const float* x_t, const float* image, const int32_t* t_original, float* logits_out,
                       int32_t B, void* workspace, void* stream) {
  TRY(check_call(p, B, workspace));
  if (!x_t || !image || !logits_out || !t_original) return fail(DUNET_E_INVALID, "NULL tensor argument");
  cudaStream_t st = static_cast<cudaStream_t>(stream);
  uint8_t* ws = static_cast<uint8_t*>(workspace);
  const WsLayout L = ws_layout(p, B);
  int row = -1;
  bool shared = true;
  for (int n = 0; n < B; ++n) {
    if (t_original[n] < 0) return fail(DUNET_E_INVALID, "timestep %d of sample %d is negative", (int)t_original[n], n);
    shared = shared && t_original[n] == t_original[0];
  }
  if (shared)
    for (int i = 0; i < p->n_steps; ++i)
      if (p->tmap[i] == t_original[0]) row = i;
  BiasRef temb;
  if (row >= 0) {
    temb.p = p->temb_table + (size_t)row * p->temb_row;
  } else {
    const int slot = p->t_slot;
    p->t_slot = (slot + 1) % dunet_plan::T_RING;
    CUDA_TRY(cudaEventSynchronize(p->t_ev[slot]));
    int* h = p->h_t + (size_t)slot * p->cfg.batch_max;
    for (int n = 0; n < B; ++n) h[n] = t_original[n];
    CUDA_TRY(cudaMemcpyAsync(p->d_t, h, (size_t)B * sizeof(int), cudaMemcpyHostToDevice, st));
    CUDA_TRY(cudaEventRecord(p->t_ev[slot], st));
    TRY(launch_temb(p, p->d_t, B, p->temb_scratch, st));
    temb.p = p->temb_scratch;
    temb.n_stride = p->temb_row;
  }
  TRY(launch_pack(p, x_t, p->C, image, p->cfg.in_channels, ws_act(p, ws, L.in_pack, p->in_pad, 0, B), p->in_pad, p->V[0], B, st));
  int nseg = 0;
  Act feat;
  TRY(unet_body(p, temb, B, ws, L, st, &nseg, &feat));
  FinalDdimArgs a;
  final_args_common(p, a, ws, L, nseg, B, feat);
  a.image = image; a.logits_out = logits_out;
  a.r = 1.f; a.m = 1.f; a.abp = 1.f;
  return launch_final(p, a, st);
}

struct NoiseSrc {
  const float* given = nullptr;
  unsigned long long seed = 0;
  const int64_t* ids = nullptr;
  int draw = 0;
};

static int ddim_core(dunet_plan* p, const float* image, const NoiseSrc& nz, int id0, float* per_step_logits, size_t per_step_stride,
                     int B, int run_encoder, int zero_acc, uint8_t* ws, cudaStream_t st) {
  const WsLayout L = ws_layout(p, B);
  const int CP = p->C <= 8 ? 8 : (p->C <= 16 ? 16 : 32);
  float* x_t = reinterpret_cast<float*>(ws + L.x_t);
  float* acc = reinterpret_cast<float*>(ws + L.acc);
  if (run_encoder) TRY(encode_impl(p, image, B, ws, L, st));
  const Act in_pack = ws_act(p, ws, L.in_pack, p->in_pad, 0, B);
  for (int b0 = 0; b0 < B; b0 += INIT_MAX_B) {
    const int nb = std::min(INIT_MAX_B, B - b0);
    DdimInitArgs ia;
    memset(&ia, 0, sizeof ia);
    ia.noise = nz.given ? nz.given + (size_t)b0 * p->C * p->V[0] : nullptr;
    ia.image = image + (size_t)b0 * p->V[0];
    ia.x_t = x_t + (size_t)b0 * p->V[0] * CP; ia.acc = acc + (size_t)b0 * p->V[0] * CP;
    ia.next_in = in_pack.hi + (size_t)b0 * p->in_pad * p->V[0];
    ia.next_in_lo = in_pack.lo ? in_pack.lo + (size_t)b0 * p->in_pad * p->V[0] : nullptr;
    ia.C = p->C; ia.CP = CP; ia.in_pad = p->in_pad; ia.batch = nb; ia.zero_acc = zero_acc; ia.vox = p->V[0]; ia.seed = nz.seed;
    for (int j = 0; j < nb; ++j) ia.ids[j] = nz.ids ? (long long)(((unsigned long long)nz.ids[id0 + b0 + j] & 0xFFFFFFFFFFull) | ((unsigned long long)nz.draw << 40)) : 0;
    const int nch = std::max(CP, p->in_pad) / 8;
    if (PROF_ON) prof_of(p)->bytes[PROF_GLUE] += (double)nb * p->V[0] * (CP * 8.0 + p->in_pad * 2.0 + 4.0 + (nz.given ? 4.0 * p->C : 0.0));
    TRY(prof_begin(PROF_GLUE, st));
    DUNET_FMT(fmt_h(p, in_pack.lo != nullptr), launch_k(ddim_init_kernel<HF>, dim3(grid_for((long long)nb * p->V[0] * nch, 256, 148 * 8)), dim3(256), 0, st, ia));
    LAUNCH_CHECK();
    TRY(prof_end(st));
  }
  for (int i = p->n_steps - 1, k = 0; i >= 0; --i, ++k) {
    int nseg = 0;
    Act feat;
    BiasRef temb;
    temb.p = p->temb_table + (size_t)i * p->temb_row;
    TRY(unet_body(p, temb, B, ws, L, st, &nseg, &feat));
    FinalDdimArgs a;
    final_args_common(p, a, ws, L, nseg, B, feat);
    a.image = image; a.x_t = x_t; a.acc = acc;
    a.logits_out = per_step_logits ? per_step_logits + (size_t)k * per_step_stride : nullptr;
    a.next_in = i > 0 ? in_pack.hi : nullptr;
    a.next_in_lo = i > 0 ? in_pack.lo : nullptr;
    a.r = p->sr[i]; a.m = p->srm1[i]; a.abp = p->acp[i];
    TRY(launch_final(p, a, st));
  }
  return 0;
}

static int ddim_sample_impl(dunet_plan* p, const float* image, const float* noise, float* acc_out, float* per_step_logits,
                            size_t per_step_stride, float* final_x, int B, int run_encoder, float out_scale, int out_accumulate,
                            uint8_t* ws, cudaStream_t st) {
  NoiseSrc nz;
  nz.given = noise;
  TRY(ddim_core(p, image, nz, 0, per_step_logits, per_step_stride, B, run_encoder, 1, ws, st));
  const WsLayout L = ws_layout(p, B);
  const int CP = p->C <= 8 ? 8 : (p->C <= 16 ? 16 : 32);
  const int sgrid = grid_for((long long)B * p->V[0] * (CP / 4), 256, 148 * 8);
  TRY(prof_begin(PROF_GLUE, st));
  launch_k(state_from_vm_kernel, dim3(sgrid), dim3(256), 0, st, (const float*)(ws + L.acc), acc_out, p->C, CP, (long long)p->V[0], B, out_scale,
           out_accumulate);
  LAUNCH_CHECK();
  TRY(prof_end(st));
  if (final_x) {
    launch_k(state_from_vm_kernel, dim3(sgrid), dim3(256), 0, st, (const float*)(ws + L.x_t), final_x, p->C, CP, (long long)p->V[0], B, 1.f, 0);
    LAUNCH_CHECK();
  }
  return 0;
}

int dunet_ddim_sample(dunet_plan* p, const float* image, const float* noise, float* acc_out, float* per_step_logits,
                      float* final_x, int32_t B, int32_t run_encoder, float out_scale, int32_t out_accumulate, void* workspace,
                      void* stream) {
  TRY(check_call(p, B, workspace));
  if (!image || !noise || !acc_out) return fail(DUNET_E_INVALID, "NULL tensor argument");
  if (!aligned16(image) || !aligned16(noise) || !aligned16(acc_out)) return fail(DUNET_E_INVALID, "tensors must be 16-byte aligned");
  cudaStream_t st = static_cast<cudaStream_t>(stream);
  uint8_t* ws = static_cast<uint8_t*>(workspace);
  const size_t per_step_stride = (size_t)B * p->C * p->V[0];
  const SubBatches s = sub_batches(p, B, use_dual(p, B, run_encoder));
  return run_sub_batches(p, s, B, ws, st, [&](int b0, int nb, uint8_t* ws_h, cudaStream_t sh) -> int {
    const size_t img_off = (size_t)b0 * p->cfg.in_channels * p->V[0], st_off = (size_t)b0 * p->C * p->V[0];
    return ddim_sample_impl(p, image + img_off, noise + st_off, acc_out + st_off, per_step_logits ? per_step_logits + st_off : nullptr,
                            per_step_stride, final_x ? final_x + st_off : nullptr, nb, run_encoder, out_scale, out_accumulate, ws_h, sh);
  });
}

static int check_box(const int32_t v[3], const int32_t pd[3], const int32_t s[3]) {
  for (int d = 0; d < 3; ++d)
    if (pd[d] < 1 || v[d] < 1 || s[d] < 0 || s[d] + pd[d] > v[d])
      return fail(DUNET_E_INVALID, "window [%d, %d) outside volume extent %d on axis %d", s[d], s[d] + pd[d], v[d], d);
  return 0;
}

int dunet_crop_window(const float* volume, const int32_t v[3], float* patch, const int32_t pd[3], const int32_t s[3], void* stream) {
  if (!volume || !patch || !v || !pd || !s) return fail(DUNET_E_INVALID, "NULL argument");
  TRY(check_box(v, pd, s));
  crop_window_kernel<<<grid_for((long long)pd[0] * pd[1] * pd[2], 256), 256, 0, static_cast<cudaStream_t>(stream)>>>(
      volume, patch, v[0], v[1], v[2], pd[0], pd[1], pd[2], s[0], s[1], s[2]);
  LAUNCH_CHECK();
  return 0;
}

static int crop_batch(const dunet_plan* p, const float* volume, const int32_t v[3], float* patches, const int32_t pd[3],
                      const int32_t* starts, int B, cudaStream_t st) {
  const long long pv = (long long)pd[0] * pd[1] * pd[2];
  for (int b0 = 0; b0 < B; b0 += INIT_MAX_B) {
    const int nb = std::min(INIT_MAX_B, B - b0);
    CropArgs c;
    memset(&c, 0, sizeof c);
    c.vol = volume; c.patches = patches + (size_t)b0 * pv;
    c.VD = v[0]; c.VH = v[1]; c.VW = v[2]; c.PD = pd[0]; c.PH = pd[1]; c.PW = pd[2]; c.batch = nb;
    for (int j = 0; j < nb; ++j) {
      TRY(check_box(v, pd, starts + 3 * (b0 + j)));
      for (int d = 0; d < 3; ++d) c.start[j][d] = starts[3 * (b0 + j) + d];
    }
    if (p) {
      if (PROF_ON) prof_of(p)->bytes[PROF_GLUE] += 8.0 * nb * pv;
      TRY(prof_begin(PROF_GLUE, st));
    }
    launch_k(crop_windows_kernel, dim3(grid_for(pv * nb, 256)), dim3(256), 0, st, c);
    LAUNCH_CHECK();
    if (p) TRY(prof_end(st));
// ... 208 lines not shown
                      uint64_t* counts, void* stream) {
  if (!pred || !label || !counts || channels < 1 || voxels < 1) return fail(DUNET_E_INVALID, "bad argument");
  cudaStream_t st = static_cast<cudaStream_t>(stream);
  CUDA_TRY(cudaMemsetAsync(counts, 0, (size_t)channels * 3 * sizeof(uint64_t), st));
  const dim3 grid(grid_for(voxels, 256, 148 * 8 / std::max(1, std::min(channels, 8))), channels);
  if (label_is_float)
    dice_counts_kernel<float><<<grid, 256, 0, st>>>(pred, static_cast<const float*>(label), (long long)voxels,
                                                    reinterpret_cast<unsigned long long*>(counts));
  else
    dice_counts_kernel<uint8_t><<<grid, 256, 0, st>>>(pred, static_cast<const uint8_t*>(label), (long long)voxels,
                                                      reinterpret_cast<unsigned long long*>(counts));
  LAUNCH_CHECK();
  return 0;
}

int dunet_hd95_workspace_bytes(int32_t channels, const int32_t dims[3], size_t* out_bytes) {
  TRY(hd95_check_dims(channels, dims));
  if (!out_bytes) return fail(DUNET_E_INVALID, "out_bytes is NULL");
  *out_bytes = hd95_layout(dims).total;
  return 0;
}

int dunet_hd95(const uint8_t* pred, const void* label, int32_t label_is_float, int32_t channels, const int32_t dims[3],
               const double spacing[3], double* hd95_out, void* workspace, size_t workspace_bytes, void* stream) {
  TRY(hd95_check_dims(channels, dims));
  if (!pred || !label || !spacing || !hd95_out || !workspace) return fail(DUNET_E_INVALID, "NULL argument");
  if ((label_is_float && (reinterpret_cast<uintptr_t>(label) & 3u)) || (reinterpret_cast<uintptr_t>(hd95_out) & 7u))
    return fail(DUNET_E_INVALID, "label (fp32) must be 4-byte and hd95_out 8-byte aligned");
  if (reinterpret_cast<uintptr_t>(workspace) & 255u) return fail(DUNET_E_INVALID, "workspace must be 256-byte aligned");
  for (int d = 0; d < 3; ++d)
    if (!std::isfinite(spacing[d]) || !(spacing[d] > 0.0)) return fail(DUNET_E_INVALID, "spacing[%d] must be finite and > 0", d);
  const Hd95Layout L = hd95_layout(dims);
  if (workspace_bytes < L.total) return fail(DUNET_E_INVALID, "workspace of %zu bytes, %zu needed", workspace_bytes, L.total);
  const HdGeom g{dims[0], dims[1], dims[2], spacing[0], spacing[1], spacing[2]};
  const size_t V = (size_t)dims[0] * dims[1] * dims[2];
  cudaStream_t st = static_cast<cudaStream_t>(stream);
  char* ws = static_cast<char*>(workspace);
  for (int c = 0; c < channels; ++c) {
    if (label_is_float)
      TRY(hd95_class(pred + c * V, static_cast<const float*>(label) + c * V, g, ws, L, hd95_out + c, st));
    else
      TRY(hd95_class(pred + c * V, static_cast<const uint8_t*>(label) + c * V, g, ws, L, hd95_out + c, st));
  }
  return 0;
}

int dunet_op_conv3x3x3(const float* src0, int32_t c0, const float* src1, int32_t c1, const float* weight, int32_t cout,
                       float* out, int32_t B, const int32_t dims[3], int32_t use_ref, void* stream) {
  if (!src0 || !weight || !out || !dims || c0 < 1 || cout < 1 || B < 1) return fail(DUNET_E_INVALID, "bad argument");
  if (c1 > 0 && !src1) return fail(DUNET_E_INVALID, "src1 is NULL but c1 > 0");
  if (use_ref < 0 || use_ref > 6) return fail(DUNET_E_INVALID, "use_ref_kernel must be 0..6");
  cudaStream_t st = static_cast<cudaStream_t>(stream);
  const bool prec = use_ref == 3 || use_ref == 4, fp16 = use_ref >= 5;
  const bool generic_only = use_ref == 2 || use_ref == 4 || use_ref == 6;
  dunet_plan tmp;
  memset(&tmp.cfg, 0, sizeof tmp.cfg);
  TRY(dev_prepare(&tmp.num_sms));
  tmp.cfg.flags = use_ref == 1 ? (DUNET_FLAG_REF_CONV | DUNET_FLAG_KEEP_FP32_WEIGHTS) : (prec ? DUNET_FLAG_FP32X3 : (fp16 ? DUNET_FLAG_FP16 : 0));
  if (generic_only) tmp.cfg.flags |= DUNET_FLAG_GENERIC_CONV;
  tmp.D[0] = dims[0]; tmp.H[0] = dims[1]; tmp.W[0] = dims[2];
  tmp.V[0] = (long long)dims[0] * dims[1] * dims[2];
  ConvW c;
  const bool small = (c1 == 0 && c0 <= 32);
  c.shape(c0, small ? 32 : pad_to(c0, 64), c1, c1 > 0 ? pad_to(c1, 64) : 0, cout, prec ? 3 : 1);
  if (c1 > 0 && (c0 % 8)) return fail(DUNET_E_UNSUPPORTED, "concat needs c0 %% 8 == 0");
  const long long vox = tmp.V[0];
  const size_t pm = prec ? 2 : 1;
  Act a0, a1, raw;
  CUDA_TRY(cudaMallocAsync((void**)&a0.hi, pm * B * c.c0p * vox * sizeof(bf16), st));
  CUDA_TRY(cudaMallocAsync((void**)&raw.hi, pm * B * c.coutp * vox * sizeof(bf16), st));
  if (prec) { a0.lo = a0.hi + (size_t)B * c.c0p * vox; raw.lo = raw.hi + (size_t)B * c.coutp * vox; }
  TRY(launch_pack(&tmp, src0, c0, nullptr, 0, a0, c.c0p, vox, B, st));
  if (c1 > 0) {
    CUDA_TRY(cudaMallocAsync((void**)&a1.hi, pm * B * c.c1p * vox * sizeof(bf16), st));
    if (prec) a1.lo = a1.hi + (size_t)B * c.c1p * vox;
    TRY(launch_pack(&tmp, src1, c1, nullptr, 0, a1, c.c1p, vox, B, st));
  }
  int rc = 0;
  if (use_ref == 1) {
    c.w32 = const_cast<float*>(weight);
  } else {
    CUDA_TRY(cudaMallocAsync((void**)&c.packed, c.packed_elems() * sizeof(bf16), st));
    pack_conv_w_kernel<<<grid_for((long long)c.packed_elems(), 256), 256, 0, st>>>(
        weight, c.packed, c.coutr, c0 + c1, c.c0r, c.c0p, c.c1r, c.cb_ch, c.n_tile, c.ncb(), c.n_tiles, 0, c.parts, fp16 ? 1 : 0, 0);
    LAUNCH_CHECK();
    if (c.coutp == 64 && !generic_only) {
      const size_t n64 = c.packed64_elems();
      CUDA_TRY(cudaMallocAsync((void**)&c.packed64, n64 * sizeof(bf16), st));
      pack_conv_w64_kernel<<<grid_for((long long)n64, 256), 256, 0, st>>>(weight, c.packed64, c.coutr, c0 + c1, c.c0r, c.c0p,
                                                                           c.c1r, c.cb64, c.ncb64(), 0, c.parts, fp16 ? 1 : 0, 0);
      LAUNCH_CHECK();
    }
  }
  int nseg_unused = 0;
  rc = run_conv(&tmp, c, conv_plan(&tmp, c, 0, false), a0, a1, raw, nullptr, nullptr, &nseg_unused, 0, B, st);
  if (rc == 0) {
    DUNET_FMT(fp16, unpack_c8_kernel<HF><<<grid_for((long long)B * (c.coutp / 8) * vox, 256), 256, 0, st>>>(raw.hi, raw.lo, c.coutp, out, cout, vox, B));
    g_launches.fetch_add(1);
    if (cudaGetLastError() != cudaSuccess) rc = fail(DUNET_E_CUDA, "unpack launch failed");
  }
  cudaFreeAsync(a0.hi, st);
  cudaFreeAsync(raw.hi, st);
  if (a1.hi) cudaFreeAsync(a1.hi, st);
  if (c.packed) cudaFreeAsync(c.packed, st);
  if (c.packed64) cudaFreeAsync(c.packed64, st);
  return rc;
}

int dunet_op_deconv2x2x2(const float* src, int32_t cin, const float* weight, const float* bias, int32_t cout, float* out,
                         int32_t B, const int32_t dims[3], int32_t use_ref, void* stream) {
  if (!src || !weight || !bias || !out || !dims || cin < 1 || cout < 1 || B < 1) return fail(DUNET_E_INVALID, "bad argument");
  if (use_ref < 0 || use_ref > 6) return fail(DUNET_E_INVALID, "use_ref_kernel must be 0..6");
  cudaStream_t st = static_cast<cudaStream_t>(stream);
  const bool prec = use_ref == 3 || use_ref == 4, fp16 = use_ref >= 5;
  dunet_plan tmp;
  memset(&tmp.cfg, 0, sizeof tmp.cfg);
  TRY(dev_prepare(&tmp.num_sms));
  tmp.cfg.flags = use_ref == 1 ? DUNET_FLAG_REF_CONV : ((use_ref == 2 || use_ref == 4 || use_ref == 6) ? DUNET_FLAG_GENERIC_CONV : 0);
  if (prec) tmp.cfg.flags |= DUNET_FLAG_FP32X3;
  if (fp16) tmp.cfg.flags |= DUNET_FLAG_FP16;
  tmp.D[0] = dims[0]; tmp.H[0] = dims[1]; tmp.W[0] = dims[2];
  tmp.V[0] = (long long)dims[0] * dims[1] * dims[2];
  DeconvW d;
  d.cinr = cin; d.cinp = pad_to(cin, 64); d.coutr = cout; d.coutp = pad_to(cout, 64); d.parts = prec ? 3 : 1;
  const long long vox = tmp.V[0];
  const size_t nw = 8ull * d.cinp * d.coutp;
  const size_t pm = prec ? 2 : 1;
  Act a0, o;
  CUDA_TRY(cudaMallocAsync((void**)&a0.hi, pm * B * d.cinp * vox * sizeof(bf16), st));
  CUDA_TRY(cudaMallocAsync((void**)&o.hi, pm * B * d.coutp * vox * 8 * sizeof(bf16), st));
  if (prec) { a0.lo = a0.hi + (size_t)B * d.cinp * vox; o.lo = o.hi + (size_t)B * d.coutp * vox * 8; }
  CUDA_TRY(cudaMallocAsync((void**)&d.packed, nw * sizeof(bf16), st));
  CUDA_TRY(cudaMallocAsync((void**)&d.packed_tc, nw * d.parts * sizeof(bf16), st));
  CUDA_TRY(cudaMallocAsync((void**)&d.bias, d.coutp * sizeof(float), st));
  TRY(launch_pack(&tmp, src, cin, nullptr, 0, a0, d.cinp, vox, B, st));
  pack_deconv_w_kernel<<<grid_for((long long)nw, 256), 256, 0, st>>>(weight, d.packed, cin, cout, d.cinp, d.coutp, fp16 ? 1 : 0);
  LAUNCH_CHECK();
  pack_deconv_tc_w_kernel<<<grid_for((long long)nw * d.parts, 256), 256, 0, st>>>(weight, d.packed_tc, cin, cout, d.cinp, d.coutp, d.parts, fp16 ? 1 : 0);
  LAUNCH_CHECK();
  copy_pad_rows_kernel<<<1, 256, 0, st>>>(bias, d.bias, 1, cout, 1, d.coutp);
  LAUNCH_CHECK();
  int rc = run_deconv(&tmp, d, a0, o, 0, B, st);
  if (rc == 0) {
    DUNET_FMT(fp16, unpack_c8_kernel<HF><<<grid_for((long long)B * (d.coutp / 8) * vox * 8, 256), 256, 0, st>>>(o.hi, o.lo, d.coutp, out, cout, vox * 8, B));
    g_launches.fetch_add(1);
    if (cudaGetLastError() != cudaSuccess) rc = fail(DUNET_E_CUDA, "unpack launch failed");
  }
  cudaFreeAsync(a0.hi, st); cudaFreeAsync(o.hi, st); cudaFreeAsync(d.packed, st); cudaFreeAsync(d.packed_tc, st); cudaFreeAsync(d.bias, st);
  return rc;
}

int dunet_debug_conv_geometry(const int32_t dims[3], int32_t cin, int32_t cout, uint32_t flags, int32_t out[16]) {
  if (!dims || !out || cin < 1 || cout < 1 || dims[0] < 1 || dims[1] < 1 || dims[2] < 1) return fail(DUNET_E_INVALID, "bad argument");
  dunet_plan tmp;
  memset(&tmp.cfg, 0, sizeof tmp.cfg);
  tmp.cfg.flags = flags;
  tmp.D[0] = dims[0]; tmp.H[0] = dims[1]; tmp.W[0] = dims[2];
  tmp.V[0] = (long long)dims[0] * dims[1] * dims[2];
  ConvW c;
  c.shape(cin, cin <= 32 ? 32 : pad_to(cin, 64), 0, 0, cout, (flags & DUNET_FLAG_FP32X3) ? 3 : 1);
  const ConvPlan g = conv_plan(&tmp, c, 0, true);
  out[0] = g.kernel == CONV_TC64 ? 0 : (g.kernel == CONV_FLAT ? 2 : 1);
  out[1] = g.zt; out[2] = g.tiles_x; out[3] = g.tiles_y; out[4] = g.tiles_z; out[5] = g.ksplit; out[6] = g.ksub;
  out[7] = g.flat.hx; out[8] = g.flat.ty; out[9] = g.flat.npos; out[10] = g.flat.a_slots; out[11] = g.flat.w_slots; out[12] = g.flat.smem;
  out[13] = g.tiles * c.n_tiles; out[14] = c.n_tiles; out[15] = c.ncb();
  return 0;
}

int dunet_debug_set_conv_timeline(int64_t* dev_buffer) {
  g_conv_dbg = reinterpret_cast<long long*>(dev_buffer);
  g_conv_dbg_count = 0;
  return 0;
}
// ... 3 lines not shown
```

### diff-unet-amos_b200/csrc/elementwise.cuh

```cuda
#pragma once
#include <cstdint>
#include <cuda_bf16.h>
#include <cuda_fp16.h>
#include <cuda_runtime.h>

#include "ptx.cuh"

namespace dunet {

struct alignas(16) BF8 {
  __nv_bfloat162 v[4];
};

template <bool H>
__device__ __forceinline__ void bf8_to_float(const BF8& b, float (&f)[8]) {
#pragma unroll
  for (int i = 0; i < 4; ++i) {
    float2 t;
    if constexpr (H) t = __half22float2(*reinterpret_cast<const __half2*>(&b.v[i]));
    else t = __bfloat1622float2(b.v[i]);
    f[2 * i] = t.x;
    f[2 * i + 1] = t.y;
  }
}
template <bool H>
__device__ __forceinline__ BF8 float_to_bf8(const float (&f)[8]) {
  BF8 b;
#pragma unroll
  for (int i = 0; i < 4; ++i) {
    if constexpr (H) *reinterpret_cast<__half2*>(&b.v[i]) = __floats2half2_rn(f[2 * i], f[2 * i + 1]);
    else b.v[i] = __floats2bfloat162_rn(f[2 * i], f[2 * i + 1]);
  }
  return b;
}
template <bool H>
__device__ __forceinline__ uint32_t pack_16x2(float lo, float hi) {
  if constexpr (H) {
    __half2 v = __floats2half2_rn(lo, hi);
    return *reinterpret_cast<uint32_t*>(&v);
  } else {
    __nv_bfloat162 v = __floats2bfloat162_rn(lo, hi);
    return *reinterpret_cast<uint32_t*>(&v);
  }
}
template <bool H>
__device__ __forceinline__ float2 unpack_16x2(uint32_t w) {
  if constexpr (H) return __half22float2(*reinterpret_cast<const __half2*>(&w));
  else return __bfloat1622float2(*reinterpret_cast<const __nv_bfloat162*>(&w));
}
template <bool H>
__device__ __forceinline__ float round_16(float v) {
  if constexpr (H) return __half2float(__float2half_rn(v));
  else return __bfloat162float(__float2bfloat16_rn(v));
}

template <bool H>
__device__ __forceinline__ void store_split(__nv_bfloat16* hi, __nv_bfloat16* lo, long long idx8, const float (&f)[8]) {
  const BF8 h = float_to_bf8<H>(f);
  reinterpret_cast<BF8*>(hi)[idx8] = h;
  if constexpr (!H) {
    if (lo) {
      float hf[8], r[8];
      bf8_to_float<false>(h, hf);
#pragma unroll
      for (int j = 0; j < 8; ++j) r[j] = f[j] - hf[j];
      reinterpret_cast<BF8*>(lo)[idx8] = float_to_bf8<false>(r);
    }
  }
}
template <bool H>
__device__ __forceinline__ void load_split(const __nv_bfloat16* hi, const __nv_bfloat16* lo, long long idx8, float (&f)[8]) {
  bf8_to_float<H>(reinterpret_cast<const BF8*>(hi)[idx8], f);
  if constexpr (!H) {
    if (lo) {
      float g[8];
      bf8_to_float<false>(reinterpret_cast<const BF8*>(lo)[idx8], g);
#pragma unroll
      for (int j = 0; j < 8; ++j) f[j] += g[j];
    }
  }
}

template <bool H>
__global__ void pack_c8_kernel(const float* __restrict__ src0, int c0, const float* __restrict__ src1, int c1,
                               __nv_bfloat16* __restrict__ dst, __nv_bfloat16* __restrict__ dst_lo, int c_pad, long long vox,
                               int batch, int triple) {
  pdl_wait();
  const int chunks = c_pad / 8;
  long long total = (long long)batch * chunks * vox;
  for (long long i = blockIdx.x * (long long)blockDim.x + threadIdx.x; i < total;
       i += (long long)gridDim.x * blockDim.x) {
    long long v = i % vox;
    int ck = (int)((i / vox) % chunks);
    int n = (int)(i / (vox * chunks));
    float f[8];
#pragma unroll
    for (int j = 0; j < 8; ++j) {
      int c = ck * 8 + j;
      float val = 0.f;
      if (triple) {
        if (c < 3 * c0) {
          const float x = src0[((long long)n * c0 + c % c0) * vox + v];
          const float hi = round_16<false>(x);
          val = (c / c0 == 1) ? x - hi : hi;
        }
      } else if (c < c0) val = src0[((long long)n * c0 + c) * vox + v];
      else if (c < c0 + c1) val = src1[((long long)n * c1 + (c - c0)) * vox + v];
      f[j] = val;
    }
    store_split<H>(dst, triple ? nullptr : dst_lo, i, f);
  }
}

template <bool H>
__global__ void unpack_c8_kernel(const __nv_bfloat16* __restrict__ src, const __nv_bfloat16* __restrict__ src_lo, int c_pad,
                                 float* __restrict__ dst, int c_out, long long vox, int batch) {
  const int chunks = c_pad / 8;
  long long total = (long long)batch * chunks * vox;
  for (long long i = blockIdx.x * (long long)blockDim.x + threadIdx.x; i < total;
       i += (long long)gridDim.x * blockDim.x) {
    long long v = i % vox;
    int ck = (int)((i / vox) % chunks);
    int n = (int)(i / (vox * chunks));
    float f[8];
    load_split<H>(src, src_lo, i, f);
#pragma unroll
    for (int j = 0; j < 8; ++j) {
      int c = ck * 8 + j;
      if (c < c_out) dst[((long long)n * c_out + c) * vox + v] = f[j];
    }
  }
}

constexpr int STATS_THREADS = 256;

template <bool H>
__global__ void __launch_bounds__(STATS_THREADS) in_stats_kernel(const __nv_bfloat16* __restrict__ raw,
                                                                 float* __restrict__ partial, long long vox, int nseg) {
  const int plane = blockIdx.y, seg = blockIdx.x;
  const BF8* p = reinterpret_cast<const BF8*>(raw) + (long long)plane * vox;
  long long per = (vox + nseg - 1) / nseg;
  long long lo = seg * per, hi = min(vox, lo + per);
  float s[8], q[8];
#pragma unroll
  for (int j = 0; j < 8; ++j) s[j] = q[j] = 0.f;
  for (long long v = lo + threadIdx.x; v < hi; v += STATS_THREADS) {
    float f[8];
    bf8_to_float<H>(p[v], f);
#pragma unroll
    for (int j = 0; j < 8; ++j) {
      s[j] += f[j];
      q[j] = fmaf(f[j], f[j], q[j]);
    }
  }
  __shared__ float red[STATS_THREADS / 32][16];
#pragma unroll
  for (int j = 0; j < 8; ++j) {
#pragma unroll
    for (int o = 16; o > 0; o >>= 1) {
      s[j] += __shfl_xor_sync(0xffffffffu, s[j], o);
      q[j] += __shfl_xor_sync(0xffffffffu, q[j], o);
    }
  }
  const int warp = threadIdx.x >> 5, lane = threadIdx.x & 31;
  if (lane == 0) {
#pragma unroll
    for (int j = 0; j < 8; ++j) {
      red[warp][j] = s[j];
      red[warp][8 + j] = q[j];
    }
  }
  __syncthreads();
  if (threadIdx.x < 16) {
    float t = 0.f;
    for (int w = 0; w < STATS_THREADS / 32; ++w) t += red[w][threadIdx.x];
    partial[((long long)plane * nseg + seg) * 16 + threadIdx.x] = t;
  }
}

template <bool H>
__global__ void __launch_bounds__(STATS_THREADS) splitk_reduce_stats_kernel(const float* __restrict__ part, int ksplit,
                                                                            long long split_stride ,
                                                                            __nv_bfloat16* __restrict__ raw,
                                                                            __nv_bfloat16* __restrict__ raw_lo,
                                                                            float* __restrict__ partial, long long vox,
                                                                            int nseg) {
  pdl_wait();
  const int plane = blockIdx.y, seg = blockIdx.x;
  const float4* p = reinterpret_cast<const float4*>(part) + (long long)plane * vox * 2;
  long long per = (vox + nseg - 1) / nseg;
  long long lo = seg * per, hi = min(vox, lo + per);
  float s[8], q[8];
#pragma unroll
// ... 415 lines not shown
      norm_apply(f[u], sc, sh, bi, a.n.slope);
      if constexpr (ADD) {
        float g[8];
        bf8_to_float<H>(add[v], g);
#pragma unroll
        for (int j = 0; j < 8; ++j) f[u][j] += g[j];
      }
      const BF8 o = float_to_bf8<H>(f[u]);
      out[v] = o;
      if constexpr (POOL) tile[v] = o;
    }
  }
  if constexpr (POOL) {
    __syncthreads();
    const int D2 = a.n.D / 2, H2 = a.n.H / 2, W2 = a.n.W / 2;
    const int pvox = D2 * H2 * W2;
    for (int pv = threadIdx.x; pv < pvox; pv += 256) {
      const int x2 = pv % W2, y2 = (pv / W2) % H2, z2 = pv / (W2 * H2);
      float m[8];
#pragma unroll
      for (int j = 0; j < 8; ++j) m[j] = -INFINITY;
#pragma unroll
      for (int k = 0; k < 8; ++k) {
        float r[8];
        bf8_to_float<H>(tile[((2 * z2 + (k >> 2)) * a.n.H + 2 * y2 + ((k >> 1) & 1)) * a.n.W + 2 * x2 + (k & 1)], r);
#pragma unroll
        for (int j = 0; j < 8; ++j) m[j] = fmaxf(m[j], r[j]);
      }
      store_split<H>(a.n.pooled, nullptr, (long long)plane * pvox + pv, m);
    }
  }
}

template <bool HF>
__global__ void __launch_bounds__(256) deconv2_kernel(const __nv_bfloat16* __restrict__ in, int cin,
                                                      const __nv_bfloat16* __restrict__ w, const float* __restrict__ b,
                                                      __nv_bfloat16* __restrict__ out, int cout, int D, int H, int W,
                                                      int batch) {
  const long long vox = (long long)D * H * W;
  const int och = cout / 8, ich = cin / 8;
  const long long total = (long long)batch * och * 8 * vox;
  for (long long i = blockIdx.x * (long long)blockDim.x + threadIdx.x; i < total;
       i += (long long)gridDim.x * blockDim.x) {
    const long long v = i % vox;
    const int tap = (int)((i / vox) % 8);
    const int oc = (int)((i / (vox * 8)) % och);
    const int n = (int)(i / (vox * 8 * och));
    float acc[8];
#pragma unroll
    for (int j = 0; j < 8; ++j) acc[j] = b[oc * 8 + j];
    const BF8* ip = reinterpret_cast<const BF8*>(in) + (long long)n * ich * vox + v;
    const BF8* wp = reinterpret_cast<const BF8*>(w) + ((long long)tap * cin) * och + oc;
    for (int ic = 0; ic < ich; ++ic) {
      float xi[8];
      bf8_to_float<HF>(ip[(long long)ic * vox], xi);
#pragma unroll
      for (int k = 0; k < 8; ++k) {
        float wk[8];
        bf8_to_float<HF>(wp[(long long)(ic * 8 + k) * och], wk);
#pragma unroll
        for (int j = 0; j < 8; ++j) acc[j] = fmaf(xi[k], wk[j], acc[j]);
      }
    }
    const int x = (int)(v % W), y = (int)((v / W) % H), z = (int)(v / ((long long)W * H));
    const int dz = tap >> 2, dy = (tap >> 1) & 1, dx = tap & 1;
    const long long ov = ((long long)(2 * z + dz) * (2 * H) + (2 * y + dy)) * (2 * W) + (2 * x + dx);
    reinterpret_cast<BF8*>(out)[((long long)n * och + oc) * (vox * 8) + ov] = float_to_bf8<HF>(acc);
  }
}

struct FinalDdimArgs {
  const __nv_bfloat16* feat;
  const __nv_bfloat16* feat_lo;
  __nv_bfloat16* next_in_lo;
  int F;
  const float* partial;
  int nseg;
  const float* gamma;
  const float* beta;
  float eps, slope;
  const float* w;
  const float* b;
  int C;
  const float* image;
  float* x_t;
  float* acc;
  float* logits_out;
  __nv_bfloat16* next_in;
  int in_pad;
  long long vox;
  int batch;
  float r, m, abp;
};

constexpr int FINAL_MAX_C = 32;
constexpr int FINAL_MAX_F = 128;
constexpr int FINAL_THREADS = 256;

template <bool H>
__device__ __forceinline__ void mma_16816(float (&d)[4], const uint32_t (&a)[4], uint32_t b0, uint32_t b1) {
  if constexpr (H)
    asm volatile("mma.sync.aligned.m16n8k16.row.col.f32.f16.f16.f32 {%0,%1,%2,%3}, {%4,%5,%6,%7}, {%8,%9}, {%0,%1,%2,%3};"
                 : "+f"(d[0]), "+f"(d[1]), "+f"(d[2]), "+f"(d[3])
                 : "r"(a[0]), "r"(a[1]), "r"(a[2]), "r"(a[3]), "r"(b0), "r"(b1));
  else
    asm volatile("mma.sync.aligned.m16n8k16.row.col.f32.bf16.bf16.f32 {%0,%1,%2,%3}, {%4,%5,%6,%7}, {%8,%9}, {%0,%1,%2,%3};"
                 : "+f"(d[0]), "+f"(d[1]), "+f"(d[2]), "+f"(d[3])
                 : "r"(a[0]), "r"(a[1]), "r"(a[2]), "r"(a[3]), "r"(b0), "r"(b1));
}

template <int NT, int NKS, int MODE>
__global__ void __launch_bounds__(FINAL_THREADS) final_ddim_kernel(FinalDdimArgs a) {
  constexpr bool PREC = MODE == MODE_FP32X3, H = MODE == MODE_FP16;
  __shared__ uint32_t wfrag[(FINAL_MAX_F / 16) * NT * 2 * 2 * 32];
  __shared__ float sbias[NT * 8];
  __shared__ __align__(8) float nsc[FINAL_MAX_F], nsh[FINAL_MAX_F];
  __shared__ double scratch[4 * 256];
  constexpr int nks = NKS;
  const int fch = a.F / 8;
  const int n = blockIdx.y;
  const int lane = threadIdx.x & 31, g = lane >> 2, t = lane & 3;
  for (int i = threadIdx.x; i < nks * NT * 32; i += FINAL_THREADS) {
    const int l = i & 31, nt = (i >> 5) % NT, ks = i / (32 * NT);
    const int cls = nt * 8 + (l >> 2), k0 = ks * 16 + 2 * (l & 3);
    float wv[4];
#pragma unroll
    for (int j = 0; j < 4; ++j) {
      const int k = k0 + (j & 1) + (j >> 1) * 8;
      wv[j] = cls < a.C ? a.w[cls * a.F + k] : 0.f;
    }
    float hi[4], lo[4];
#pragma unroll
    for (int j = 0; j < 4; ++j) {
      hi[j] = round_16<H>(wv[j]);
      lo[j] = wv[j] - hi[j];
    }
    uint32_t* dst = wfrag + ((ks * NT + nt) * 4) * 32 + l;
    dst[0] = pack_16x2<H>(hi[0], hi[1]);
    dst[32] = pack_16x2<H>(hi[2], hi[3]);
    dst[64] = pack_16x2<H>(lo[0], lo[1]);
    dst[96] = pack_16x2<H>(lo[2], lo[3]);
  }
  for (int i = threadIdx.x; i < NT * 8; i += FINAL_THREADS) sbias[i] = i < a.C ? a.b[i] : 0.f;
  pdl_wait();
  if (a.partial) stats_to_affine_planes(a.partial, a.nseg, n * fch, fch, a.gamma, a.beta, fch, (double)a.vox, a.eps, nsc, nsh, scratch);
  __syncthreads();

  const float s_abp = sqrtf(a.abp), s_1mabp = sqrtf(1.f - a.abp - 0.f);
  const unsigned vox = (unsigned)a.vox;
  const uint32_t* __restrict__ fw = reinterpret_cast<const uint32_t*>(a.feat) + (size_t)n * fch * vox * 4 + t;
  const uint32_t* __restrict__ fw_lo = reinterpret_cast<const uint32_t*>(a.feat_lo) + (size_t)n * fch * vox * 4 + t;
  const float* __restrict__ img_n = a.image ? a.image + (size_t)n * vox : nullptr;
  float2* xt_n = a.x_t ? reinterpret_cast<float2*>(a.x_t) + (size_t)n * vox * (NT * 4) + t : nullptr;
  float2* acc_n = a.acc ? reinterpret_cast<float2*>(a.acc) + (size_t)n * vox * (NT * 4) + t : nullptr;
  float* lg_n = a.logits_out ? a.logits_out + (size_t)n * a.C * vox : nullptr;
  uint32_t* np_n = a.next_in ? reinterpret_cast<uint32_t*>(a.next_in) + (size_t)n * (a.in_pad / 8) * vox * 4 + t : nullptr;
  uint32_t* np_lo_n = (PREC && a.next_in) ? reinterpret_cast<uint32_t*>(a.next_in_lo) + (size_t)n * (a.in_pad / 8) * vox * 4 + t : nullptr;
  unsigned cls_off[NT][2];
  bool cls_ok[NT][2], cls_img[NT][2];
#pragma unroll
  for (int nt = 0; nt < NT; ++nt)
#pragma unroll
    for (int b = 0; b < 2; ++b) {
      const int cls = nt * 8 + 2 * t + b;
      cls_ok[nt][b] = cls < a.C;
      cls_img[nt][b] = cls == a.C;
      cls_off[nt][b] = (unsigned)cls * vox;
    }
  const unsigned warps = gridDim.x * (FINAL_THREADS / 32);
  const unsigned warp_id = blockIdx.x * (FINAL_THREADS / 32) + (threadIdx.x >> 5);
  const unsigned ngroups = (vox + 15) / 16;
  for (unsigned grp = warp_id; grp < ngroups; grp += warps) {
    const unsigned v0 = grp * 16 + g, v1 = v0 + 8;
    const bool ok0 = v0 < vox, ok1 = v1 < vox;
    float2 xt[NT][2], ac[NT][2];
    if (xt_n) {
#pragma unroll
      for (int nt = 0; nt < NT; ++nt) {
        xt[nt][0] = ok0 ? xt_n[v0 * (NT * 4) + nt * 4] : make_float2(0.f, 0.f);
        xt[nt][1] = ok1 ? xt_n[v1 * (NT * 4) + nt * 4] : make_float2(0.f, 0.f);
        ac[nt][0] = ok0 ? acc_n[v0 * (NT * 4) + nt * 4] : make_float2(0.f, 0.f);
        ac[nt][1] = ok1 ? acc_n[v1 * (NT * 4) + nt * 4] : make_float2(0.f, 0.f);
      }
    }
    const float img0 = (np_n && ok0) ? img_n[v0] : 0.f;
    const float img1 = (np_n && ok1) ? img_n[v1] : 0.f;
    uint32_t af[NKS][4], al[PREC ? NKS : 1][4];
#pragma unroll
    for (int ks = 0; ks < NKS; ++ks) {
      const unsigned c0 = (2 * ks) * vox, c1 = c0 + vox;
      af[ks][0] = ok0 ? __ldg(fw + (c0 + v0) * 4) : 0u;
      af[ks][1] = ok1 ? __ldg(fw + (c0 + v1) * 4) : 0u;
      af[ks][2] = ok0 ? __ldg(fw + (c1 + v0) * 4) : 0u;
      af[ks][3] = ok1 ? __ldg(fw + (c1 + v1) * 4) : 0u;
      if constexpr (PREC) {
        al[ks][0] = ok0 ? __ldg(fw_lo + (c0 + v0) * 4) : 0u;
        al[ks][1] = ok1 ? __ldg(fw_lo + (c0 + v1) * 4) : 0u;
        al[ks][2] = ok0 ? __ldg(fw_lo + (c1 + v0) * 4) : 0u;
        al[ks][3] = ok1 ? __ldg(fw_lo + (c1 + v1) * 4) : 0u;
      }
    }
    float d[NT][4];
#pragma unroll
    for (int nt = 0; nt < NT; ++nt) {
      d[nt][0] = d[nt][2] = sbias[nt * 8 + 2 * t];
      d[nt][1] = d[nt][3] = sbias[nt * 8 + 2 * t + 1];
    }
#pragma unroll
    for (int ks = 0; ks < NKS; ++ks) {
      if (a.partial) {
#pragma unroll
        for (int j = 0; j < 4; ++j) {
          const int c = ks * 16 + (j >> 1) * 8 + 2 * t;
          float2 x = unpack_16x2<H>(af[ks][j]);
          if constexpr (PREC) {
            const float2 xl = unpack_16x2<false>(al[ks][j]);
            x.x += xl.x; x.y += xl.y;
          }
          const float2 sc2 = *reinterpret_cast<const float2*>(nsc + c), sh2 = *reinterpret_cast<const float2*>(nsh + c);
          float y0 = fmaf(x.x, sc2.x, sh2.x), y1 = fmaf(x.y, sc2.y, sh2.y);
          y0 = fmaxf(y0, y0 * a.slope);
          y1 = fmaxf(y1, y1 * a.slope);
          af[ks][j] = pack_16x2<H>(y0, y1);
          if constexpr (PREC) {
            const float2 h = unpack_16x2<false>(af[ks][j]);
            al[ks][j] = pack_16x2<false>(y0 - h.x, y1 - h.y);
          }
        }
      }
#pragma unroll
      for (int nt = 0; nt < NT; ++nt) {
        const uint32_t* wf = wfrag + ((ks * NT + nt) * 4) * 32 + lane;
        mma_16816<H>(d[nt], af[ks], wf[0], wf[32]);
        mma_16816<H>(d[nt], af[ks], wf[64], wf[96]);
        if constexpr (PREC) mma_16816<false>(d[nt], al[ks], wf[0], wf[32]);
      }
    }
#pragma unroll
    for (int nt = 0; nt < NT; ++nt) {
      float nxt[4];
      float xp4[4], ac4[4];
#pragma unroll
      for (int j = 0; j < 4; ++j) {
        const bool okv = (j >> 1) ? ok1 : ok0;
        const float xin = (j & 1) ? xt[nt][j >> 1].y : xt[nt][j >> 1].x;
        const float ain = (j & 1) ? ac[nt][j >> 1].y : ac[nt][j >> 1].x;
        float val = cls_img[nt][j & 1] ? ((j >> 1) ? img1 : img0) : 0.f;
        xp4[j] = 0.f;
        ac4[j] = 0.f;
        if (cls_ok[nt][j & 1] && okv) {
          const float lg = d[nt][j];
          if (lg_n) lg_n[cls_off[nt][j & 1] + ((j >> 1) ? v1 : v0)] = lg;
          if (xt_n) {
            const float x0 = fminf(fmaxf(lg, -1.f), 1.f);
            const float eps = (a.r * xin - x0) / a.m;
            const float xp = x0 * s_abp + s_1mabp * eps;
            xp4[j] = xp;
            ac4[j] = ain + x0;
            val = xp;
          }
        }
        nxt[j] = val;
      }
      if (xt_n) {
        if (ok0) { xt_n[v0 * (NT * 4) + nt * 4] = make_float2(xp4[0], xp4[1]); acc_n[v0 * (NT * 4) + nt * 4] = make_float2(ac4[0], ac4[1]); }
        if (ok1) { xt_n[v1 * (NT * 4) + nt * 4] = make_float2(xp4[2], xp4[3]); acc_n[v1 * (NT * 4) + nt * 4] = make_float2(ac4[2], ac4[3]); }
      }
      if (np_n && nt * 8 < a.in_pad) {
        const uint32_t h0 = pack_16x2<H>(nxt[0], nxt[1]), h1 = pack_16x2<H>(nxt[2], nxt[3]);
        if (ok0) np_n[(nt * vox + v0) * 4] = h0;
        if (ok1) np_n[(nt * vox + v1) * 4] = h1;
        if constexpr (PREC) {
          const float2 f0 = unpack_16x2<false>(h0), f1 = unpack_16x2<false>(h1);
          if (ok0) np_lo_n[(nt * vox + v0) * 4] = pack_16x2<false>(nxt[0] - f0.x, nxt[1] - f0.y);
          if (ok1) np_lo_n[(nt * vox + v1) * 4] = pack_16x2<false>(nxt[2] - f1.x, nxt[3] - f1.y);
        }
      }
    }
  }
}

__global__ void state_from_vm_kernel(const float* __restrict__ src, float* __restrict__ dst, int C, int CP, long long vox, int batch,
                                     float scale, int accumulate) {
  pdl_wait();
  const int q4 = CP / 4;
  const long long total = (long long)batch * vox * q4;
  for (long long i = blockIdx.x * (long long)blockDim.x + threadIdx.x; i < total; i += (long long)gridDim.x * blockDim.x) {
    const int qd = (int)(i % q4);
    const long long v = (i / q4) % vox;
    const int n = (int)(i / (q4 * vox));
    const float4 f4 = reinterpret_cast<const float4*>(src)[i];
    const float f[4] = {f4.x, f4.y, f4.z, f4.w};
#pragma unroll
    for (int j = 0; j < 4; ++j) {
      const int c = qd * 4 + j;
      if (c < C) {
        float* o = dst + ((long long)n * C + c) * vox + v;
        *o = accumulate ? fmaf(scale, f[j], *o) : scale * f[j];
      }
    }
  }
}

__device__ __forceinline__ void philox4x32_10(uint32_t (&c)[4], uint32_t k0, uint32_t k1) {
#pragma unroll
  for (int r = 0; r < 10; ++r) {
    const uint32_t hi0 = __umulhi(0xD2511F53u, c[0]), lo0 = 0xD2511F53u * c[0];
    const uint32_t hi1 = __umulhi(0xCD9E8D57u, c[2]), lo1 = 0xCD9E8D57u * c[2];
    const uint32_t n0 = hi1 ^ c[1] ^ k0, n2 = hi0 ^ c[3] ^ k1;
    c[0] = n0; c[1] = lo1; c[2] = n2; c[3] = lo0;
    k0 += 0x9E3779B9u; k1 += 0xBB67AE85u;
  }
}
__device__ __forceinline__ void box_muller(uint32_t a, uint32_t b, float& z0, float& z1) {
  const float u1 = ((float)(a >> 8) + 1.0f) * (1.0f / 16777216.0f);
  const float u2 = (float)(b >> 8) * (1.0f / 16777216.0f);
  const float r = sqrtf(-2.0f * __logf(u1));
  float sn, cs;
  __sincosf(6.283185307179586f * u2, &sn, &cs);
  z0 = r * cs;
  z1 = r * sn;
}
constexpr int INIT_MAX_B = 16;
struct DdimInitArgs {
  const float* noise;
  const float* image;
  float* x_t;
  float* acc;
  __nv_bfloat16* next_in;
  __nv_bfloat16* next_in_lo;
  int C, CP, in_pad, batch, zero_acc;
  long long vox;
  unsigned long long seed;
  long long ids[INIT_MAX_B];
};
template <bool H>
__global__ void __launch_bounds__(256) ddim_init_kernel(DdimInitArgs a) {
  pdl_wait();
  const int nch = (a.CP > a.in_pad ? a.CP : a.in_pad) / 8;
  const long long total = (long long)a.batch * a.vox * nch;
  for (long long i = blockIdx.x * (long long)blockDim.x + threadIdx.x; i < total; i += (long long)gridDim.x * blockDim.x) {
    const int ck = (int)(i % nch);
    const long long v = (i / nch) % a.vox;
    const int n = (int)(i / (nch * a.vox));
    float f[8];
    if (a.noise) {
#pragma unroll
      for (int j = 0; j < 8; ++j) {
        const int c = ck * 8 + j;
        f[j] = c < a.C ? a.noise[((long long)n * a.C + c) * a.vox + v] : 0.f;
      }
    } else {
      const unsigned long long e = (unsigned long long)v * (unsigned)(a.CP / 4) + (unsigned)(ck * 2);
      const unsigned long long id = (unsigned long long)a.ids[n];
#pragma unroll
      for (int h = 0; h < 2; ++h) {
        uint32_t c4[4] = {(uint32_t)(e + h), (uint32_t)((e + h) >> 32), (uint32_t)id, (uint32_t)(id >> 32)};
        philox4x32_10(c4, (uint32_t)a.seed, (uint32_t)(a.seed >> 32));
        box_muller(c4[0], c4[1], f[4 * h + 0], f[4 * h + 1]);
        box_muller(c4[2], c4[3], f[4 * h + 2], f[4 * h + 3]);
      }
#pragma unroll
      for (int j = 0; j < 8; ++j)
        if (ck * 8 + j >= a.C) f[j] = 0.f;
    }
    if (ck * 8 < a.CP) {
      float4* xs = reinterpret_cast<float4*>(a.x_t + ((long long)n * a.vox + v) * a.CP + ck * 8);
      xs[0] = make_float4(f[0], f[1], f[2], f[3]);
      xs[1] = make_float4(f[4], f[5], f[6], f[7]);
      if (a.zero_acc) {
        float4* as = reinterpret_cast<float4*>(a.acc + ((long long)n * a.vox + v) * a.CP + ck * 8);
        as[0] = make_float4(0.f, 0.f, 0.f, 0.f);
        as[1] = make_float4(0.f, 0.f, 0.f, 0.f);
      }
    }
    if (ck * 8 < a.in_pad) {
      if (a.C >= ck * 8 && a.C < ck * 8 + 8) f[a.C - ck * 8] = a.image[(long long)n * a.vox + v];
      store_split<H>(a.next_in, a.next_in_lo, ((long long)n * (a.in_pad / 8) + ck) * a.vox + v, f);
    }
  }
}

__global__ void __launch_bounds__(256) q_sample_kernel(const float* __restrict__ x0, const float* __restrict__ noise_in,
                                                       float* __restrict__ noise_out, const long long* __restrict__ t,
                                                       const float* __restrict__ sqrt_ac, const float* __restrict__ sqrt_1mac,
                                                       float* __restrict__ out, long long per_sample, int batch,
                                                       unsigned long long seed, long long id0) {
  const long long groups = (per_sample + 3) / 4;
  const long long total = groups * batch;
  for (long long i = blockIdx.x * (long long)blockDim.x + threadIdx.x; i < total; i += (long long)gridDim.x * blockDim.x) {
    const int n = (int)(i / groups);
    const long long g = i % groups;
    const float a = sqrt_ac[t[n]], b = sqrt_1mac[t[n]];
    float z[4];
    if (!noise_in) {
      const unsigned long long id = (unsigned long long)(id0 + n);
      uint32_t c4[4] = {(uint32_t)g, (uint32_t)((unsigned long long)g >> 32), (uint32_t)id, (uint32_t)(id >> 32)};
      philox4x32_10(c4, (uint32_t)seed, (uint32_t)(seed >> 32));
      box_muller(c4[0], c4[1], z[0], z[1]);
      box_muller(c4[2], c4[3], z[2], z[3]);
    }
#pragma unroll
    for (int j = 0; j < 4; ++j) {
      const long long e = g * 4 + j;
      if (e < per_sample) {
        const long long o = (long long)n * per_sample + e;
        const float nz = noise_in ? noise_in[o] : z[j];
        if (noise_out) noise_out[o] = nz;
        out[o] = __fadd_rn(__fmul_rn(a, x0[o]), __fmul_rn(b, nz));
      }
    }
  }
}

struct CropArgs {
  const float* vol;
  float* patches;
  int VD, VH, VW, PD, PH, PW, batch;
  int start[INIT_MAX_B][3];
};
__global__ void crop_windows_kernel(CropArgs a) {
  pdl_wait();
  const long long pv = (long long)a.PD * a.PH * a.PW;
  const long long total = pv * a.batch;
  for (long long i = blockIdx.x * (long long)blockDim.x + threadIdx.x; i < total; i += (long long)gridDim.x * blockDim.x) {
    const int b = (int)(i / pv);
    const long long r = i % pv;
    const int x = (int)(r % a.PW), y = (int)((r / a.PW) % a.PH), z = (int)(r / ((long long)a.PW * a.PH));
    a.patches[i] = a.vol[((long long)(a.start[b][0] + z) * a.VH + a.start[b][1] + y) * a.VW + a.start[b][2] + x];
  }
}

__global__ void __launch_bounds__(256) stitch_from_vm_kernel(float* __restrict__ vol, float* __restrict__ cnt,
                                                             const float* __restrict__ acc_vm, const float* __restrict__ w,
                                                             int C, int CP, int VD, int VH, int VW, int PD, int PH, int PW,
                                                             int sz, int sy, int sx, float scale) {
  pdl_wait();
  const long long pv = (long long)PD * PH * PW, vv = (long long)VD * VH * VW;
  for (long long v = blockIdx.x * (long long)blockDim.x + threadIdx.x; v < pv; v += (long long)gridDim.x * blockDim.x) {
    const int x = (int)(v % PW), y = (int)((v / PW) % PH), z = (int)(v / ((long long)PW * PH));
    const long long o = ((long long)(sz + z) * VH + sy + y) * VW + sx + x;
    const float4* src = reinterpret_cast<const float4*>(acc_vm + v * CP);
    const float wv = w ? w[v] : 1.f;
    for (int q = 0; q < CP / 4; ++q) {
      const float4 f4 = src[q];
      const float f[4] = {f4.x, f4.y, f4.z, f4.w};
#pragma unroll
      for (int j = 0; j < 4; ++j) {
        const int c = q * 4 + j;
        if (c < C) {
          const float pred = scale == 1.f ? f[j] : __fmul_rn(scale, f[j]);
          float* dst = vol + c * vv + o;
          *dst = w ? __fadd_rn(*dst, __fmul_rn(wv, pred)) : __fadd_rn(*dst, pred);
        }
      }
    }
    if (w) cnt[o] = __fadd_rn(cnt[o], wv);
  }
}

// ... 292 lines not shown
```

Measured before the change: 77.54.

## Fold image channel 3x3 taps into channels and skip empty K-steps in first conv

The static image input channel of the network's first conv is expanded into 9 (or 27 for split precision) shifted in-plane copies packed as extra channels, so its weights only need the centre tap. A SPARSE variant of the tc64 conv kernel uses per-block K-step masks to skip MMA issues and weight loads for the zero K-steps of the non-centre taps. This cuts tensor-core work on the image channel at the cost of a wider packed input and more complex packing in ddim_init and a new pack_first kernel. The final DDIM kernel no longer writes the image channel into the next step's input.

```diff
diff --git a/diff-unet-amos_b200/csrc/conv3d_ref.cuh b/diff-unet-amos_b200/csrc/conv3d_ref.cuh
--- a/diff-unet-amos_b200/csrc/conv3d_ref.cuh
+++ b/diff-unet-amos_b200/csrc/conv3d_ref.cuh
@@ -11,7 +11,7 @@
                                                          const __nv_bfloat16* __restrict__ src1, int c1, int chunks1,
                                                          const float* __restrict__ w ,
                                                          __nv_bfloat16* __restrict__ out, int cout, int out_chunks,
-                                                         int D, int H, int W, int batch, int rot) {
+                                                         int D, int H, int W, int batch, int img_ch) {
   const long long vox = (long long)D * H * W;
   const int och = (cout + 7) / 8;
   const int cin = c0 + c1;
@@ -36,6 +36,17 @@
           if (xx < 0 || xx >= W) continue;
           const int tap = (tz * 3 + ty) * 3 + tx;
           const long long sv = ((long long)zz * H + yy) * W + xx;
+          if (img_ch >= 0) {
+            for (int ci = 0; ci < c0; ++ci) {
+              const int pc = ci == 0 ? img_ch + 4 : ci - 1;
+              float xi[8];
+              bf8_to_float<HF>(reinterpret_cast<const BF8*>(src0)[((long long)n * chunks0 + pc / 8) * vox + sv], xi);
+#pragma unroll
+              for (int j = 0; j < 8; ++j)
+                if (oc * 8 + j < cout) acc[j] = fmaf(xi[pc % 8], round_16<HF>(w[((long long)(oc * 8 + j) * cin + ci) * 27 + tap]), acc[j]);
+            }
+            continue;
+          }
           for (int ci = 0; ci < cin; ci += 8) {
             const bool second = ci >= c0;
             const BF8* sp = second ? reinterpret_cast<const BF8*>(src1) + ((long long)n * chunks1 + (ci - c0) / 8) * vox
@@ -49,7 +60,7 @@
                 for (int j = 0; j < 8; ++j) {
                   if (oc * 8 + j >= cout) continue;
                   const float wv =
-                      round_16<HF>(w[((long long)(oc * 8 + j) * cin + (rot ? (ci + k + 1) % c0 : ci + k)) * 27 + tap]);
+                      round_16<HF>(w[((long long)(oc * 8 + j) * cin + ci + k) * 27 + tap]);
                   acc[j] = fmaf(xi[k], wv, acc[j]);
                 }
               }
diff --git a/diff-unet-amos_b200/csrc/conv3d_tc64.cuh b/diff-unet-amos_b200/csrc/conv3d_tc64.cuh
--- a/diff-unet-amos_b200/csrc/conv3d_tc64.cuh
+++ b/diff-unet-amos_b200/csrc/conv3d_tc64.cuh
@@ -18,6 +18,7 @@
   static constexpr int A_LBO = HY * HX * 16, A_SBO = HX * 16;
   static constexpr int NROWS = 192;
   static constexpr int W_UNIT_BYTES = KCH * NROWS * 16;
+  static constexpr int W_KSTEP_BYTES = 2 * NROWS * 16;
   static constexpr int B_LBO = NROWS * 16, B_SBO = 128;
   static constexpr int PLANES = ZT + 2;
   static constexpr int A_SLOTS = CB_CH == 32 ? 2 * PLANES + 1 : PLANES + 1;
@@ -40,6 +41,8 @@
   ConvSegs segs;
   int D, H, W;
   int tiles_x, tiles_y, tiles_z, batch;
+  uint32_t k_all, k_ctr;
+  int kblocks;
   const float* in_affine;
   const float* in_bias;
   int in_bias_n_stride;
@@ -55,7 +58,19 @@
   }
 }
 
-template <int CB_CH, int ZT, bool FUSE, bool H>
+template <int KC, bool SPARSE>
+__device__ __forceinline__ void block_ksteps(const ConvTc64Args& a, int cb, uint32_t& all, uint32_t& ctr) {
+  if constexpr (SPARSE) {
+    const int sh = (cb % a.kblocks) * KC;
+    all = (a.k_all >> sh) & ((1u << KC) - 1u);
+    ctr = (a.k_ctr >> sh) & ((1u << KC) - 1u);
+  } else {
+    all = (1u << KC) - 1u;
+    ctr = 0;
+  }
+}
+
+template <int CB_CH, int ZT, bool FUSE, bool H, bool SPARSE = false>
 __global__ void __launch_bounds__(FUSE ? ConvTc64<CB_CH, ZT>::THREADS_FUSED : CONV_THREADS, 1)
 conv3d_tc64_kernel(const __grid_constant__ CUtensorMap tmap0, const __grid_constant__ CUtensorMap tmap1,
                    const __grid_constant__ CUtensorMap tmap2, const __grid_constant__ CUtensorMap tmap3, ConvTc64Args a) {
@@ -129,13 +144,22 @@
     if (elect_one_sync()) {
       int w = 0;
       for_each_tile(tiles_per_n, a.batch, [&](int, int) {
-        for (int i = 0; i < ncb * 9; ++i, ++w) {
-          const int slot = w % Cfg::W_SLOTS, it = w / Cfg::W_SLOTS;
-          if (it > 0) mbar_wait(w_empty + 8 * slot, (it - 1) & 1);
-          mbar_arrive_expect_tx(w_full + 8 * slot, Cfg::W_UNIT_BYTES);
-          bulk_load_1d(w_smem + slot * Cfg::W_UNIT_BYTES,
-                       reinterpret_cast<const uint8_t*>(a.w) + (size_t)i * Cfg::W_UNIT_BYTES, Cfg::W_UNIT_BYTES,
-                       w_full + 8 * slot);
+        for (int cb = 0; cb < ncb; ++cb) {
+          uint32_t all, ctr;
+          block_ksteps<Cfg::KC, SPARSE>(a, cb, all, ctr);
+          for (int tyx = 0; tyx < 9; ++tyx) {
+            const uint32_t km = tyx == 4 ? all | ctr : all;
+            if (!km) continue;
+            const int k0 = __ffs(km) - 1, k1 = 31 - __clz(km);
+            const int off = k0 * Cfg::W_KSTEP_BYTES, bytes = (k1 - k0 + 1) * Cfg::W_KSTEP_BYTES;
+            const int slot = w % Cfg::W_SLOTS, it = w / Cfg::W_SLOTS;
+            if (it > 0) mbar_wait(w_empty + 8 * slot, (it - 1) & 1);
+            mbar_arrive_expect_tx(w_full + 8 * slot, bytes);
+            bulk_load_1d(w_smem + slot * Cfg::W_UNIT_BYTES + off,
+                         reinterpret_cast<const uint8_t*>(a.w) + (size_t)(cb * 9 + tyx) * Cfg::W_UNIT_BYTES + off, bytes,
+                         w_full + 8 * slot);
+            ++w;
+          }
         }
       });
     }
@@ -152,6 +176,8 @@
         if (use > 0) { mbar_wait(acc_empty + 8 * buf, (use - 1) & 1); tc_fence_after(); }
         const uint32_t acc = tmem_base + buf * Cfg::ACC_COLS;
         for (int cb = 0; cb < ncb; ++cb, u0 += Cfg::PLANES) {
+          uint32_t k_all, k_ctr;
+          block_ksteps<Cfg::KC, SPARSE>(a, cb, k_all, k_ctr);
           uint32_t pl_lo[Cfg::PLANES], pl_bar[Cfg::PLANES];
           uint32_t par[Cfg::PLANES];
 #pragma unroll
@@ -163,6 +189,9 @@
           }
           auto tap = [&](auto kind, int tyx, bool first_cb) {
             constexpr int KIND = decltype(kind)::value;
+            constexpr bool FIRST = (KIND & 1) != 0, LAST = (KIND & 2) != 0;
+            const uint32_t km = SPARSE ? (tyx == 4 ? k_all | k_ctr : k_all) : (1u << Cfg::KC) - 1u;
+            const int k_init = SPARSE ? __ffs(km) - 1 : 0;
             const int ws = w & (Cfg::W_SLOTS - 1);
             mbar_wait(w_full + 8 * ws, (w / Cfg::W_SLOTS) & 1);
             tc_fence_after();
@@ -170,19 +199,19 @@
             const uint32_t bl_u = b_lo0 + ws * (Cfg::W_UNIT_BYTES >> 4);
 #pragma unroll
             for (int p = 0; p < Cfg::PLANES; ++p) {
-              if constexpr (KIND == 0) {
+              if constexpr (FIRST) {
                 mbar_wait((FUSE ? a_ready : a_full) + pl_bar[p], par[p]);
                 tc_fence_after();
               }
-              constexpr int dummy = 0; (void)dummy;
               const int slab_lo = p >= 2 ? p - 2 : 0, slab_hi = p < ZT ? p : ZT - 1;
               const int nblk = slab_hi - slab_lo + 1;
               const int row0 = (2 - (p - slab_lo)) * 64;
               const uint32_t al_p = pl_lo[p] + tap16, bl_p = bl_u + row0;
 #pragma unroll
               for (int k = 0; k < Cfg::KC; ++k) {
+                if (SPARSE && !(km >> k & 1u)) continue;
                 const uint32_t al = al_p + k * 2 * (Cfg::A_LBO >> 4), bl = bl_p + k * 2 * (Cfg::B_LBO >> 4);
-                if (KIND == 0 && k == 0 && first_cb) {
+                if (FIRST && first_cb && k == k_init) {
 #pragma unroll
                   for (int i = 0; i < nblk; ++i) {
                     const int sl = slab_lo + i, tz = p - sl;
@@ -192,15 +221,19 @@
                   umma_bf16_lh(acc + slab_lo * 64, al, a_hi, bl, b_hi, make_idesc_16(128, 64 * nblk, H), 1u);
                 }
               }
-              if constexpr (KIND == 2) umma_commit(a_empty + pl_bar[p]);
+              if constexpr (LAST) umma_commit(a_empty + pl_bar[p]);
             }
             umma_commit(w_empty + 8 * ws);
             ++w;
           };
-          tap(std::integral_constant<int, 0>{}, 0, cb == 0);
+          if (k_all) {
+            tap(std::integral_constant<int, 1>{}, 0, cb == 0);
 #pragma unroll 1
-          for (int tyx = 1; tyx < 8; ++tyx) tap(std::integral_constant<int, 1>{}, tyx, false);
-          tap(std::integral_constant<int, 2>{}, 8, false);
+            for (int tyx = 1; tyx < 8; ++tyx) tap(std::integral_constant<int, 0>{}, tyx, false);
+            tap(std::integral_constant<int, 2>{}, 8, false);
+          } else {
+            tap(std::integral_constant<int, 3>{}, 4, cb == 0);
+          }
         }
         umma_commit(acc_full + 8 * buf);
         ++li;
diff --git a/diff-unet-amos_b200/csrc/dunet.cu b/diff-unet-amos_b200/csrc/dunet.cu
--- a/diff-unet-amos_b200/csrc/dunet.cu
+++ b/diff-unet-amos_b200/csrc/dunet.cu
@@ -164,8 +164,21 @@
   const bf16 hi = __float2bfloat16_rn(v);
   return part < 2 ? hi : __float2bfloat16_rn(v - __bfloat162float(hi));
 }
+__device__ __forceinline__ int packed_w_src(int lc, int& tyx, int& wpart, int c0r, int c0p, int c1r, int img_ch, int triple) {
+  if (img_ch >= 0) {
+    if (lc < img_ch) return lc < c0r - 1 ? lc + 1 : -1;
+    const int r = lc - img_ch, g = r / 9;
+    if (g >= (triple ? 3 : 1) || tyx != 4) return -1;
+    tyx = r % 9;
+    if (triple) wpart = g == 2 ? 2 : 0;
+    return 0;
+  }
+  if (lc < c0p) return lc < c0r ? lc : -1;
+  const int l1 = lc - c0p;
+  return l1 < c1r ? c0r + l1 : -1;
+}
 __global__ void pack_conv_w_kernel(const float* __restrict__ w, bf16* __restrict__ out, int coutr, int cinr, int c0r,
-                                   int c0p, int c1r, int cb_ch, int n_tile, int ncb, int n_tiles, int rot, int parts, int fp16, int triple) {
+                                   int c0p, int c1r, int cb_ch, int n_tile, int ncb, int n_tiles, int img_ch, int parts, int fp16, int triple) {
   const int kch = cb_ch / 8;
   const int ncb1 = ncb / parts;
   const long long total = (long long)n_tiles * ncb * 27 * kch * n_tile * 8;
@@ -180,19 +193,15 @@
     const int nt = (int)t;
     const int co = nt * n_tile + col;
     const int cb = cbg % ncb1, part = parts == 1 ? 0 : cbg / ncb1;
-    const int lc = cb * cb_ch + k * 8 + j;
-    int ci = -1, wpart = part;
-    if (triple) {
-      if (lc < 3 * c0r) { ci = lc % c0r; wpart = lc / c0r == 2 ? 2 : 0; }
-    } else if (lc < c0p) { if (lc < c0r) ci = rot ? (lc + 1) % c0r : lc; }
-    else { const int l1 = lc - c0p; if (l1 < c1r) ci = c0r + l1; }
+    int tyx = tap % 9, wpart = part;
+    const int ci = packed_w_src(cb * cb_ch + k * 8 + j, tyx, wpart, c0r, c0p, c1r, img_ch, triple);
     float v = 0.f;
-    if (co < coutr && ci >= 0) v = w[((long long)co * cinr + ci) * 27 + tap];
+    if (co < coutr && ci >= 0) v = w[((long long)co * cinr + ci) * 27 + tap / 9 * 9 + tyx];
     out[i] = weight_part(v, wpart, fp16);
   }
 }
 __global__ void pack_conv_w64_kernel(const float* __restrict__ w, bf16* __restrict__ out, int coutr, int cinr, int c0r,
-                                     int c0p, int c1r, int cb_ch, int ncb, int rot, int parts, int fp16, int triple) {
+                                     int c0p, int c1r, int cb_ch, int ncb, int img_ch, int parts, int fp16, int triple) {
   const int kch = cb_ch / 8;
   const int ncb1 = ncb / parts;
   const long long total = (long long)ncb * 9 * kch * 192 * 8;
@@ -202,19 +211,14 @@
     const int j = (int)(t % 8); t /= 8;
     const int row = (int)(t % 192); t /= 192;
     const int k = (int)(t % kch); t /= kch;
-    const int tyx = (int)(t % 9); t /= 9;
+    int tyx = (int)(t % 9); t /= 9;
     const int cbg = (int)t;
     const int cb = cbg % ncb1, part = parts == 1 ? 0 : cbg / ncb1;
     const int tz = 2 - row / 64, co = row % 64;
-    const int tap = tz * 9 + tyx;
-    const int lc = cb * cb_ch + k * 8 + j;
-    int ci = -1, wpart = part;
-    if (triple) {
-      if (lc < 3 * c0r) { ci = lc % c0r; wpart = lc / c0r == 2 ? 2 : 0; }
-    } else if (lc < c0p) { if (lc < c0r) ci = rot ? (lc + 1) % c0r : lc; }
-    else { const int l1 = lc - c0p; if (l1 < c1r) ci = c0r + l1; }
+    int wpart = part;
+    const int ci = packed_w_src(cb * cb_ch + k * 8 + j, tyx, wpart, c0r, c0p, c1r, img_ch, triple);
     float v = 0.f;
-    if (co < coutr && ci >= 0) v = w[((long long)co * cinr + ci) * 27 + tap];
+    if (co < coutr && ci >= 0) v = w[((long long)co * cinr + ci) * 27 + tz * 9 + tyx];
     out[i] = weight_part(v, wpart, fp16);
   }
 }
@@ -272,12 +276,14 @@
   bf16* packed64 = nullptr;
   float* w32 = nullptr;
   float *gamma = nullptr, *beta = nullptr;
-  int rot = 0;
+  int img_ch = -1;
+  uint32_t k_all = ~0u, k_ctr = 0;
   bool have_w = false, have_cb = false, have_g = false, have_b = false;
   void shape(int c0r_, int c0p_, int c1r_, int c1p_, int coutr_, int parts_ = 1, int cb64_ = 32) {
     c0r = c0r_; c0p = c0p_; c1r = c1r_; c1p = c1p_; coutr = coutr_; parts = parts_;
     split = parts_ == 3;
     triple = false;
+    img_ch = -1; k_all = ~0u; k_ctr = 0;
     cb64 = (c1p == 0 && c0p == 32) ? 32 : cb64_;
     coutp = pad_to(coutr, 64);
     cb_ch = (c1p == 0 && c0p == 32) ? 32 : 64;
@@ -291,6 +297,23 @@
   int ncb64() const { return (c0p + c1p) / cb64 * parts; }
   size_t packed64_elems() const { return (size_t)ncb64() * 9 * cb64 * 192; }
 };
+
+struct FirstConvLayout {
+  int x_pad, in_pad;
+  uint32_t k_all, k_ctr;
+};
+static FirstConvLayout first_conv_layout(int nx, int img_parts) {
+  FirstConvLayout f;
+  f.x_pad = pad_to(nx, 16);
+  const int img_end = f.x_pad + 9 * img_parts;
+  f.in_pad = pad_to(f.x_pad + 16 * ((9 * img_parts + 15) / 16), 32);
+  f.k_all = f.k_ctr = 0;
+  for (int s = 0; s < f.in_pad / 16; ++s) {
+    if (16 * s < f.x_pad) f.k_all |= 1u << s;
+    else if (16 * s < img_end) f.k_ctr |= 1u << s;
+  }
+  return f;
+}
 struct Act {
   bf16* hi = nullptr;
   bf16* lo = nullptr;
@@ -573,6 +596,8 @@
   X((conv3d_tc64_kernel<32, CONV_ZT, true, H>), (ConvTc64<32, CONV_ZT>::SMEM_BYTES))                           \
   X((conv3d_tc64_kernel<64, CONV_ZT, false, H>), (ConvTc64<64, CONV_ZT>::SMEM_BYTES))                          \
   X((conv3d_tc64_kernel<64, CONV_ZT, true, H>), (ConvTc64<64, CONV_ZT>::SMEM_BYTES))                           \
+  X((conv3d_tc64_kernel<32, CONV_ZT, false, H, true>), (ConvTc64<32, CONV_ZT>::SMEM_BYTES))                    \
+  X((conv3d_tc64_kernel<64, CONV_ZT, false, H, true>), (ConvTc64<64, CONV_ZT>::SMEM_BYTES))                    \
   X((deconv2_tc_kernel<1, 2, H>), (DeconvTc<1, 2>::SMEM_BYTES))                                                \
   X((deconv2_tc_kernel<2, 2, H>), (DeconvTc<2, 2>::SMEM_BYTES))                                                \
   X((conv3d_flat_kernel<1, H>), FLAT_SMEM_MAX)                                                                 \
@@ -614,11 +639,11 @@
   return 0;
 }
 
-template <int CB_CH, bool FUSE, bool H>
+template <int CB_CH, bool FUSE, bool H, bool SPARSE = false>
 static int launch_conv_tc64(const dunet_plan* p, const CUtensorMap (&t)[4], const ConvTc64Args& a, unsigned* grid_out, cudaStream_t st,
                             int conv_tag = PROF_CONV) {
   using Cfg = ConvTc64<CB_CH, CONV_ZT>;
-  auto kern = conv3d_tc64_kernel<CB_CH, CONV_ZT, FUSE, H>;
+  auto kern = conv3d_tc64_kernel<CB_CH, CONV_ZT, FUSE, H, SPARSE>;
   const long long tiles = (long long)a.tiles_x * a.tiles_y * a.tiles_z * a.batch;
   const unsigned grid = (unsigned)std::min<long long>(tiles, p->num_sms);
   *grid_out = grid;
@@ -690,7 +715,7 @@
     if (!c.w32) return fail(DUNET_E_STATE, "DUNET_FLAG_REF_CONV needs DUNET_FLAG_KEEP_FP32_WEIGHTS");
     CUDA_TRY(cudaMemsetAsync(out.hi, 0, (size_t)B * c.coutp * p->V[lvl] * sizeof(bf16), st));
     DUNET_FMT(fmt_h(p, prec), conv3d_ref_kernel<HF><<<grid_for((long long)B * ((c.coutr + 7) / 8) * p->V[lvl], 128, 148 * 64), 128, 0, st>>>(
-        src0.hi, c.c0r, c.c0p / 8, src1.hi, c.c1r, c.c1p / 8, c.w32, out.hi, c.coutr, c.coutp / 8, D, H, W, B, c.rot));
+        src0.hi, c.c0r, c.c0p / 8, src1.hi, c.c1r, c.c1p / 8, c.w32, out.hi, c.coutr, c.coutp / 8, D, H, W, B, c.img_ch));
     LAUNCH_CHECK();
     if (partial) {
       const int nseg = stats_nseg(p->V[lvl]);
@@ -726,8 +751,12 @@
       memset(&b, 0, sizeof b);
       b.w = c.packed64; b.out = out.hi; b.out_lo = out.lo; b.stats = partial; b.segs = segs;
       b.D = D; b.H = H; b.W = W; b.tiles_x = cp.tiles_x; b.tiles_y = cp.tiles_y; b.tiles_z = cp.tiles_z; b.batch = B;
+      b.k_all = c.k_all; b.k_ctr = c.k_ctr; b.kblocks = c.c0p / cp.cb;
       unsigned grid = 0;
-      if (fuse) {
+      if (c.img_ch >= 0) {
+        if (fuse) return fail(DUNET_E_STATE, "normalise-on-load requested for a network's first conv");
+        DUNET_FMT(fmt_h(p, prec), TRY(cp.cb == 32 ? (launch_conv_tc64<32, false, HF, true>(p, t, b, &grid, st, conv_tag)) : (launch_conv_tc64<64, false, HF, true>(p, t, b, &grid, st, conv_tag))));
+      } else if (fuse) {
         b.in_affine = fuse->affine; b.in_bias = fuse->bias.p; b.in_bias_n_stride = fuse->bias.n_stride; b.slope = 0.1f;
         DUNET_FMT(fmt_h(p, prec), TRY(cp.cb == 32 ? (launch_conv_tc64<32, true, HF>(p, t, b, &grid, st, conv_tag)) : (launch_conv_tc64<64, true, HF>(p, t, b, &grid, st, conv_tag))));
       } else {
@@ -1003,17 +1032,25 @@
 }
 
 static int launch_pack(const dunet_plan* p, const float* src0, int c0, const float* src1, int c1, Act dst, int c_pad,
-                       long long vox, int B, cudaStream_t st, bool triple = false) {
-  DUNET_FMT(fmt_h(p, dst.lo != nullptr || triple), launch_k(pack_c8_kernel<HF>, dim3(grid_for((long long)B * (c_pad / 8) * vox, 256)), dim3(256), 0, st,
-                                 src0, c0, src1, c1, dst.hi, dst.lo, c_pad, vox, B, triple ? 1 : 0));
+                       long long vox, int B, cudaStream_t st) {
+  DUNET_FMT(fmt_h(p, dst.lo != nullptr), launch_k(pack_c8_kernel<HF>, dim3(grid_for((long long)B * (c_pad / 8) * vox, 256)), dim3(256), 0, st,
+                                 src0, c0, src1, c1, dst.hi, dst.lo, c_pad, vox, B));
+  LAUNCH_CHECK();
+  return 0;
+}
+
+static int launch_pack_first(const dunet_plan* p, const ConvW& c, const float* x, const float* image, Act dst, int B, cudaStream_t st) {
+  DUNET_FMT(fmt_h(p, dst.lo != nullptr || c.triple), launch_k(pack_first_kernel<HF>, dim3(grid_for((long long)B * (c.c0p / 8) * p->V[0], 256)), dim3(256), 0, st,
+                                 x, c.c0r - 1, c.img_ch, image, c.triple ? 3 : 1, dst.hi, dst.lo, c.c0p, p->H[0], p->W[0], p->V[0], B));
   LAUNCH_CHECK();
   return 0;
 }
 
 static int encode_impl(dunet_plan* p, const float* image, int B, uint8_t* ws, const WsLayout& L, cudaStream_t st) {
-  const bool ep = enc_prec(p), triple = p->enc[0].a.triple;
-  const Act in_pack = ws_act_x(p, ws, L.in_pack, p->in_pad, 0, B, ep && !triple);
-  TRY(launch_pack(p, image, p->cfg.in_channels, nullptr, 0, in_pack, p->in_pad, p->V[0], B, st, triple));
+  const bool ep = enc_prec(p);
+  const ConvW& c = p->enc[0].a;
+  const Act in_pack = ws_act_x(p, ws, L.in_pack, c.c0p, 0, B, c.split && !c.triple);
+  TRY(launch_pack_first(p, c, nullptr, image, in_pack, B, st));
   for (int l = 0; l < 5; ++l) {
     const Act src = l ? ws_act_x(p, ws, L.epool[l], p->fp[l - 1], l, B, ep) : in_pack;
     const Act pooled = l < 4 ? ws_act_x(p, ws, L.epool[l + 1], p->fp[l], l + 1, B, ep) : Act();
@@ -1267,20 +1304,23 @@
     p->uoutr[l] = (l == 1) ? p->fr[5] : p->fr[l - 1];
     p->uoutp[l] = pad_to(p->uoutr[l], 64);
   }
+  const bool enc_triple = parts_enc == 3;
+  const FirstConvLayout fe = first_conv_layout(0, enc_triple ? 3 : 1), fd = first_conv_layout(p->C, 1);
+  p->in_pad = fd.in_pad;
   for (int l = 0; l < 5; ++l) {
     TwoConvW& e = p->enc[l];
     if (l == 0) {
-      e.a.shape(cfg->in_channels, p->in_pad, 0, 0, p->fr[0], parts_enc, cb64);
-      if (e.a.split && 3 * cfg->in_channels <= 32 && !(cfg->flags & DUNET_FLAG_REF_CONV)) {
-        e.a.shape(cfg->in_channels, p->in_pad, 0, 0, p->fr[0], 1, cb64);
-        e.a.split = true; e.a.triple = true;
-      }
+      e.a.shape(cfg->in_channels, fe.in_pad, 0, 0, p->fr[0], 1, cb64);
+      e.a.split = e.a.triple = enc_triple;
+      e.a.img_ch = fe.x_pad; e.a.k_all = fe.k_all; e.a.k_ctr = fe.k_ctr;
     } else e.a.shape(p->fr[l - 1], p->fp[l - 1], 0, 0, p->fr[l], parts_enc, cb64);
     e.b.shape(p->fr[l], p->fp[l], 0, 0, p->fr[l], parts_enc, cb64);
     TwoConvW& d = p->den[l];
     d.has_temb = true;
-    if (l == 0) { d.a.shape(cfg->in_channels + p->C, p->in_pad, 0, 0, p->fr[0], parts, cb64); d.a.rot = 1; }
-    else d.a.shape(p->fr[l - 1], p->fp[l - 1], 0, 0, p->fr[l], parts, cb64);
+    if (l == 0) {
+      d.a.shape(cfg->in_channels + p->C, fd.in_pad, 0, 0, p->fr[0], parts, cb64);
+      d.a.img_ch = fd.x_pad; d.a.k_all = fd.k_all; d.a.k_ctr = fd.k_ctr;
+    } else d.a.shape(p->fr[l - 1], p->fp[l - 1], 0, 0, p->fr[l], parts, cb64);
     d.b.shape(p->fr[l], p->fp[l], 0, 0, p->fr[l], parts, cb64);
   }
   for (int l = 4; l >= 1; --l) {
@@ -1351,13 +1391,13 @@
       if (!c->packed) TRY(dev_alloc(p, (void**)&c->packed, c->packed_elems() * sizeof(bf16)));
       const int cinr = c->c0r + c->c1r;
       pack_conv_w_kernel<<<grid_for((long long)c->packed_elems(), 256), 256, 0, st>>>(
-          src, c->packed, c->coutr, cinr, c->c0r, c->c0p, c->c1r, c->cb_ch, c->n_tile, c->ncb(), c->n_tiles, c->rot, c->parts, fmt_h(p, c->split) ? 1 : 0, c->triple ? 1 : 0);
+          src, c->packed, c->coutr, cinr, c->c0r, c->c0p, c->c1r, c->cb_ch, c->n_tile, c->ncb(), c->n_tiles, c->img_ch, c->parts, fmt_h(p, c->split) ? 1 : 0, c->triple ? 1 : 0);
       LAUNCH_CHECK();
       if (c->coutp == 64) {
         const size_t n64 = c->packed64_elems();
         if (!c->packed64) TRY(dev_alloc(p, (void**)&c->packed64, n64 * sizeof(bf16)));
         pack_conv_w64_kernel<<<grid_for((long long)n64, 256), 256, 0, st>>>(src, c->packed64, c->coutr, cinr, c->c0r, c->c0p,
-                                                                             c->c1r, c->cb64, c->ncb64(), c->rot, c->parts, fmt_h(p, c->split) ? 1 : 0, c->triple ? 1 : 0);
+                                                                             c->c1r, c->cb64, c->ncb64(), c->img_ch, c->parts, fmt_h(p, c->split) ? 1 : 0, c->triple ? 1 : 0);
         LAUNCH_CHECK();
       }
       if (p->cfg.flags & DUNET_FLAG_KEEP_FP32_WEIGHTS) {
@@ -1542,13 +1582,13 @@
     temb.p = p->temb_scratch;
     temb.n_stride = p->temb_row;
   }
-  TRY(launch_pack(p, x_t, p->C, image, p->cfg.in_channels, ws_act(p, ws, L.in_pack, p->in_pad, 0, B), p->in_pad, p->V[0], B, st));
+  TRY(launch_pack_first(p, p->den[0].a, x_t, image, ws_act(p, ws, L.in_pack, p->in_pad, 0, B), B, st));
   int nseg = 0;
   Act feat;
   TRY(unet_body(p, temb, B, ws, L, st, &nseg, &feat));
   FinalDdimArgs a;
   final_args_common(p, a, ws, L, nseg, B, feat);
-  a.image = image; a.logits_out = logits_out;
+  a.logits_out = logits_out;
   a.r = 1.f; a.m = 1.f; a.abp = 1.f;
   return launch_final(p, a, st);
 }
@@ -1573,11 +1613,11 @@
     DdimInitArgs ia;
     memset(&ia, 0, sizeof ia);
     ia.noise = nz.given ? nz.given + (size_t)b0 * p->C * p->V[0] : nullptr;
-    ia.image = image + (size_t)b0 * p->V[0];
+    ia.image = image + (size_t)b0 * p->V[0]; ia.H = p->H[0]; ia.W = p->W[0];
     ia.x_t = x_t + (size_t)b0 * p->V[0] * CP; ia.acc = acc + (size_t)b0 * p->V[0] * CP;
     ia.next_in = in_pack.hi + (size_t)b0 * p->in_pad * p->V[0];
     ia.next_in_lo = in_pack.lo ? in_pack.lo + (size_t)b0 * p->in_pad * p->V[0] : nullptr;
-    ia.C = p->C; ia.CP = CP; ia.in_pad = p->in_pad; ia.batch = nb; ia.zero_acc = zero_acc; ia.vox = p->V[0]; ia.seed = nz.seed;
+    ia.C = p->C; ia.CP = CP; ia.x_pad = p->den[0].a.img_ch; ia.in_pad = p->in_pad; ia.batch = nb; ia.zero_acc = zero_acc; ia.vox = p->V[0]; ia.seed = nz.seed;
     for (int j = 0; j < nb; ++j) ia.ids[j] = nz.ids ? (long long)(((unsigned long long)nz.ids[id0 + b0 + j] & 0xFFFFFFFFFFull) | ((unsigned long long)nz.draw << 40)) : 0;
     const int nch = std::max(CP, p->in_pad) / 8;
     if (PROF_ON) prof_of(p)->bytes[PROF_GLUE] += (double)nb * p->V[0] * (CP * 8.0 + p->in_pad * 2.0 + 4.0 + (nz.given ? 4.0 * p->C : 0.0));
@@ -1594,7 +1634,7 @@
     TRY(unet_body(p, temb, B, ws, L, st, &nseg, &feat));
     FinalDdimArgs a;
     final_args_common(p, a, ws, L, nseg, B, feat);
-    a.image = image; a.x_t = x_t; a.acc = acc;
+    a.x_t = x_t; a.acc = acc;
     a.logits_out = per_step_logits ? per_step_logits + (size_t)k * per_step_stride : nullptr;
     a.next_in = i > 0 ? in_pack.hi : nullptr;
     a.next_in_lo = i > 0 ? in_pack.lo : nullptr;
@@ -1969,13 +2009,13 @@
   } else {
     CUDA_TRY(cudaMallocAsync((void**)&c.packed, c.packed_elems() * sizeof(bf16), st));
     pack_conv_w_kernel<<<grid_for((long long)c.packed_elems(), 256), 256, 0, st>>>(
-        weight, c.packed, c.coutr, c0 + c1, c.c0r, c.c0p, c.c1r, c.cb_ch, c.n_tile, c.ncb(), c.n_tiles, 0, c.parts, fp16 ? 1 : 0, 0);
+        weight, c.packed, c.coutr, c0 + c1, c.c0r, c.c0p, c.c1r, c.cb_ch, c.n_tile, c.ncb(), c.n_tiles, -1, c.parts, fp16 ? 1 : 0, 0);
     LAUNCH_CHECK();
     if (c.coutp == 64 && !generic_only) {
       const size_t n64 = c.packed64_elems();
       CUDA_TRY(cudaMallocAsync((void**)&c.packed64, n64 * sizeof(bf16), st));
       pack_conv_w64_kernel<<<grid_for((long long)n64, 256), 256, 0, st>>>(weight, c.packed64, c.coutr, c0 + c1, c.c0r, c.c0p,
-                                                                           c.c1r, c.cb64, c.ncb64(), 0, c.parts, fp16 ? 1 : 0, 0);
+                                                                           c.c1r, c.cb64, c.ncb64(), -1, c.parts, fp16 ? 1 : 0, 0);
       LAUNCH_CHECK();
     }
   }
diff --git a/diff-unet-amos_b200/csrc/elementwise.cuh b/diff-unet-amos_b200/csrc/elementwise.cuh
--- a/diff-unet-amos_b200/csrc/elementwise.cuh
+++ b/diff-unet-amos_b200/csrc/elementwise.cuh
@@ -84,7 +84,7 @@
 template <bool H>
 __global__ void pack_c8_kernel(const float* __restrict__ src0, int c0, const float* __restrict__ src1, int c1,
                                __nv_bfloat16* __restrict__ dst, __nv_bfloat16* __restrict__ dst_lo, int c_pad, long long vox,
-                               int batch, int triple) {
+                               int batch) {
   pdl_wait();
   const int chunks = c_pad / 8;
   long long total = (long long)batch * chunks * vox;
@@ -98,17 +98,51 @@
     for (int j = 0; j < 8; ++j) {
       int c = ck * 8 + j;
       float val = 0.f;
-      if (triple) {
-        if (c < 3 * c0) {
-          const float x = src0[((long long)n * c0 + c % c0) * vox + v];
-          const float hi = round_16<false>(x);
-          val = (c / c0 == 1) ? x - hi : hi;
-        }
-      } else if (c < c0) val = src0[((long long)n * c0 + c) * vox + v];
+      if (c < c0) val = src0[((long long)n * c0 + c) * vox + v];
       else if (c < c0 + c1) val = src1[((long long)n * c1 + (c - c0)) * vox + v];
       f[j] = val;
     }
-    store_split<H>(dst, triple ? nullptr : dst_lo, i, f);
+    store_split<H>(dst, dst_lo, i, f);
+  }
+}
+
+__device__ __forceinline__ void image_block_chunk(const float* __restrict__ img_n, long long v, int H, int W, int r0, int parts,
+                                                  float (&f)[8]) {
+  const int x = (int)(v % W), y = (int)((v / W) % H);
+#pragma unroll
+  for (int j = 0; j < 8; ++j) {
+    const int r = r0 + j, g = r / 9, k = r % 9, dy = k / 3 - 1, dx = k % 3 - 1;
+    float val = 0.f;
+    if (r >= 0 && g < parts && y + dy >= 0 && y + dy < H && x + dx >= 0 && x + dx < W) {
+      val = img_n[v + dy * W + dx];
+      if (parts == 3) {
+        const float hi = round_16<false>(val);
+        val = g == 1 ? val - hi : hi;
+      }
+    }
+    f[j] = val;
+  }
+}
+
+template <bool H>
+__global__ void pack_first_kernel(const float* __restrict__ x, int nx, int x_pad, const float* __restrict__ image, int parts,
+                                  __nv_bfloat16* __restrict__ dst, __nv_bfloat16* __restrict__ dst_lo, int c_pad, int Hd, int Wd,
+                                  long long vox, int batch) {
+  pdl_wait();
+  const int chunks = c_pad / 8;
+  const long long total = (long long)batch * chunks * vox;
+  for (long long i = blockIdx.x * (long long)blockDim.x + threadIdx.x; i < total; i += (long long)gridDim.x * blockDim.x) {
+    const long long v = i % vox;
+    const int ck = (int)((i / vox) % chunks);
+    const int n = (int)(i / (vox * chunks));
+    float f[8];
+    if (ck * 8 < x_pad) {
+#pragma unroll
+      for (int j = 0; j < 8; ++j) f[j] = ck * 8 + j < nx ? x[((long long)n * nx + ck * 8 + j) * vox + v] : 0.f;
+    } else {
+      image_block_chunk(image + (long long)n * vox, v, Hd, Wd, ck * 8 - x_pad, parts, f);
+    }
+    store_split<H>(dst, parts == 3 ? nullptr : dst_lo, i, f);
   }
 }
 
@@ -690,7 +724,6 @@
   const float* w;
   const float* b;
   int C;
-  const float* image;
   float* x_t;
   float* acc;
   float* logits_out;
@@ -758,21 +791,19 @@
   const unsigned vox = (unsigned)a.vox;
   const uint32_t* __restrict__ fw = reinterpret_cast<const uint32_t*>(a.feat) + (size_t)n * fch * vox * 4 + t;
   const uint32_t* __restrict__ fw_lo = reinterpret_cast<const uint32_t*>(a.feat_lo) + (size_t)n * fch * vox * 4 + t;
-  const float* __restrict__ img_n = a.image ? a.image + (size_t)n * vox : nullptr;
   float2* xt_n = a.x_t ? reinterpret_cast<float2*>(a.x_t) + (size_t)n * vox * (NT * 4) + t : nullptr;
   float2* acc_n = a.acc ? reinterpret_cast<float2*>(a.acc) + (size_t)n * vox * (NT * 4) + t : nullptr;
   float* lg_n = a.logits_out ? a.logits_out + (size_t)n * a.C * vox : nullptr;
   uint32_t* np_n = a.next_in ? reinterpret_cast<uint32_t*>(a.next_in) + (size_t)n * (a.in_pad / 8) * vox * 4 + t : nullptr;
   uint32_t* np_lo_n = (PREC && a.next_in) ? reinterpret_cast<uint32_t*>(a.next_in_lo) + (size_t)n * (a.in_pad / 8) * vox * 4 + t : nullptr;
   unsigned cls_off[NT][2];
-  bool cls_ok[NT][2], cls_img[NT][2];
+  bool cls_ok[NT][2];
 #pragma unroll
   for (int nt = 0; nt < NT; ++nt)
 #pragma unroll
     for (int b = 0; b < 2; ++b) {
       const int cls = nt * 8 + 2 * t + b;
       cls_ok[nt][b] = cls < a.C;
-      cls_img[nt][b] = cls == a.C;
       cls_off[nt][b] = (unsigned)cls * vox;
     }
   const unsigned warps = gridDim.x * (FINAL_THREADS / 32);
@@ -791,8 +822,6 @@
         ac[nt][1] = ok1 ? acc_n[v1 * (NT * 4) + nt * 4] : make_float2(0.f, 0.f);
       }
     }
-    const float img0 = (np_n && ok0) ? img_n[v0] : 0.f;
-    const float img1 = (np_n && ok1) ? img_n[v1] : 0.f;
     uint32_t af[NKS][4], al[PREC ? NKS : 1][4];
 #pragma unroll
     for (int ks = 0; ks < NKS; ++ks) {
@@ -853,7 +882,7 @@
         const bool okv = (j >> 1) ? ok1 : ok0;
         const float xin = (j & 1) ? xt[nt][j >> 1].y : xt[nt][j >> 1].x;
         const float ain = (j & 1) ? ac[nt][j >> 1].y : ac[nt][j >> 1].x;
-        float val = cls_img[nt][j & 1] ? ((j >> 1) ? img1 : img0) : 0.f;
+        float val = 0.f;
         xp4[j] = 0.f;
         ac4[j] = 0.f;
         if (cls_ok[nt][j & 1] && okv) {
@@ -874,7 +903,7 @@
         if (ok0) { xt_n[v0 * (NT * 4) + nt * 4] = make_float2(xp4[0], xp4[1]); acc_n[v0 * (NT * 4) + nt * 4] = make_float2(ac4[0], ac4[1]); }
         if (ok1) { xt_n[v1 * (NT * 4) + nt * 4] = make_float2(xp4[2], xp4[3]); acc_n[v1 * (NT * 4) + nt * 4] = make_float2(ac4[2], ac4[3]); }
       }
-      if (np_n && nt * 8 < a.in_pad) {
+      if (np_n) {
         const uint32_t h0 = pack_16x2<H>(nxt[0], nxt[1]), h1 = pack_16x2<H>(nxt[2], nxt[3]);
         if (ok0) np_n[(nt * vox + v0) * 4] = h0;
         if (ok1) np_n[(nt * vox + v1) * 4] = h1;
@@ -933,11 +962,12 @@
 struct DdimInitArgs {
   const float* noise;
   const float* image;
+  int H, W;
   float* x_t;
   float* acc;
   __nv_bfloat16* next_in;
   __nv_bfloat16* next_in_lo;
-  int C, CP, in_pad, batch, zero_acc;
+  int C, CP, x_pad, in_pad, batch, zero_acc;
   long long vox;
   unsigned long long seed;
   long long ids[INIT_MAX_B];
@@ -983,7 +1013,7 @@
       }
     }
     if (ck * 8 < a.in_pad) {
-      if (a.C >= ck * 8 && a.C < ck * 8 + 8) f[a.C - ck * 8] = a.image[(long long)n * a.vox + v];
+      if (ck * 8 >= a.x_pad) image_block_chunk(a.image + (long long)n * a.vox, v, a.H, a.W, ck * 8 - a.x_pad, 1, f);
       store_split<H>(a.next_in, a.next_in_lo, ((long long)n * (a.in_pad / 8) + ck) * a.vox + v, f);
     }
   }
```

Result: no change. 77.63, median of 6 (+0.1%).
